# StavrosOrf/EV2Gym

Measured on AMD Instinct MI355X. Metric: env-steps/sec (envs x chargers x steps); % HBM roofline, higher is better.
Workload: dtype f64; 1 GPU; cfg2: V2GProfitPlusLoads, 50 chargers, 1 transformer, uniform[-1,1] actions; envs_per_gpu=4096, scenario_pool_per_gpu=32768, scenario_pool_order=sorted by busy window inside every window of envs_per_gpu scenarios, chargers=50, transformers=1, steps_per_episode=112, obs_dim=162, soc_log=True, launch=persistent, actor=none

## Files before the change

### ev2gym_amd/csrc/ev2g_device.h

```cpp
#pragma once
#include <hip/hip_runtime.h>
#include <stdint.h>

#define EV2G_BLOCK 256
#define EV2G_NQ 8

#include "ev2g_records.h"
typedef SessDyn PortDyn;

struct DevScn {
    int E;
    int M;
    int T, C, npc, P, R, D, ND, dt;
    int reward_kind, state_kind, flags, cost_kind;
    int n_lut;
    int G;
    int gs;
    int n_groups;
    double sixty_over_dt;
    double dt_over_60;
    const int *slot_port, *slot_cs, *slot_obs, *slot_tr;
    const int *cs_np, *cs_pbase, *slot_mask;
    const int *cs_slot0;
    int het;
// ... 853 lines not shown
    z = (z ^ (z >> 27)) * 0x94D049BB133111EBull;
    z = z ^ (z >> 31);
    return (double)(z >> 11) * (1.0 / 9007199254740992.0);
}

__global__ void ev2g_fill_uniform_kernel(double *dst, long long n, uint64_t seed, double lo, double hi) {
    for (long long i = blockIdx.x * (long long)blockDim.x + threadIdx.x; i < n; i += (long long)gridDim.x * blockDim.x)
        dst[i] = lo + (hi - lo) * ev2g_u01(seed, (uint64_t)i);
}

__device__ __forceinline__ double wave_sum(double v) {
    for (int d = 32; d > 0; d >>= 1) v += __shfl_xor(v, d, 64);
    return v;
}
__device__ __forceinline__ double wave_min(double v) {
    for (int d = 32; d > 0; d >>= 1) v = fmin(v, __shfl_xor(v, d, 64));
    return v;
}

__device__ __forceinline__ void port_sessions(const DevScn &s, const DevState &st, long long g, long long gs, int cur_step, int &first,
                                              int &last, bool &attached) {
    first = s.port_first[gs];
    last = first;
    attached = false;
    if (first < 0) return;
    const int2 w = make_int2(st.line[g].ta, st.line[g].td);
    const int cur = st.line[g].ss;
    if (cur < 0) {
        last = s.port_end[gs];
    } else {
        attached = (w.x <= cur_step);
        last = attached ? cur + 1 : cur;
    }
}

template <int EPWS> __device__ __forceinline__ double seg_sum(double v) {
    v += xor1_f64(v);
    v += xor2_f64(v);
    v += xor4_f64(v);
    v += dpp_mov_f64<0x128>(v);
    const int lo = __double2loint(v), hi = __double2hiint(v);
    const double r0 = __hiloint2double(__builtin_amdgcn_readlane(hi, 0), __builtin_amdgcn_readlane(lo, 0));
    const double r1 = __hiloint2double(__builtin_amdgcn_readlane(hi, 16), __builtin_amdgcn_readlane(lo, 16));
    const double r2 = __hiloint2double(__builtin_amdgcn_readlane(hi, 32), __builtin_amdgcn_readlane(lo, 32));
    const double r3 = __hiloint2double(__builtin_amdgcn_readlane(hi, 48), __builtin_amdgcn_readlane(lo, 48));
    if (EPWS == 1) return (r0 + r1) + (r2 + r3);
    return (threadIdx.x < 32) ? r0 + r1 : r2 + r3;
}
template <int EPWS> __device__ __forceinline__ double seg_min(double v) {
    v = fmin(v, xor1_f64(v));
    v = fmin(v, xor2_f64(v));
    v = fmin(v, xor4_f64(v));
    v = fmin(v, dpp_mov_f64<0x128>(v));
    const int lo = __double2loint(v), hi = __double2hiint(v);
    const double r0 = __hiloint2double(__builtin_amdgcn_readlane(hi, 0), __builtin_amdgcn_readlane(lo, 0));
    const double r1 = __hiloint2double(__builtin_amdgcn_readlane(hi, 16), __builtin_amdgcn_readlane(lo, 16));
    const double r2 = __hiloint2double(__builtin_amdgcn_readlane(hi, 32), __builtin_amdgcn_readlane(lo, 32));
    const double r3 = __hiloint2double(__builtin_amdgcn_readlane(hi, 48), __builtin_amdgcn_readlane(lo, 48));
    if (EPWS == 1) return fmin(fmin(r0, r1), fmin(r2, r3));
    return (threadIdx.x < 32) ? fmin(r0, r1) : fmin(r2, r3);
}
template <int EPWS> __device__ __forceinline__ bool seg_all(bool p) {
    const unsigned long long m = __ballot(p);
    if (EPWS == 1) return m == ~0ull;
    return (threadIdx.x < 32) ? ((unsigned)m == 0xffffffffu) : ((unsigned)(m >> 32) == 0xffffffffu);
}

struct StatsView {
    int T, C, R, P, dt;
    const double *setpoint;
    const int *scn_sess, *scn_sess_end, *ss_slot, *ss_tarr, *ss_tdep;
    const double *ss_B, *ss_afap;
    const int *cs_served;
    const double *cs_sat_sum, *hist, *env_acc, *sess_final_cap, *sess_abs_e, *soc_log;
    const PortLine *line;
};
__device__ __forceinline__ StatsView ev2g_stats_view(const DevScn &s, const DevState &st, const double *ss_afap) {
    return StatsView{s.T, s.C, s.R, s.P, s.dt, s.setpoint, s.scn_sess, s.scn_sess_end, s.ss_slot, s.ss_tarr, s.ss_tdep, s.ss_B, ss_afap,
                     st.cs_served, st.cs_sat_sum, st.hist, st.env_acc, st.sess_final_cap, st.sess_abs_e, st.soc_log, st.line};
}

#define EV2G_STATS_NK 40
#define EV2G_STATS_TB 8
#define EV2G_STATS_LK 16

template <int EPWS, int NK, int LK>
__device__ __forceinline__ void ev2g_env_stats(const StatsView &sv, int e, bool e_valid, int scn, int lane, int cur_step, double *__restrict__ out,
                                               double *l_keep, int lslot) {
    constexpr int W = 64 / EPWS;
    const int T = sv.T, C = sv.C, R = sv.R, P = sv.P;
    double served = 0.0, sat = 0.0, nsat = 0.0;
    for (int c = lane; c < C; c += W) {
        const int n = sv.cs_served[(long long)e * C + c];
        served += n;
        if (n > 0) { sat += sv.cs_sat_sum[(long long)e * C + c] / n; nsat += 1.0; }
    }
    served = seg_sum<EPWS>(served); sat = seg_sum<EPWS>(sat); nsat = seg_sum<EPWS>(nsat);
    double over = 0.0, te = 0.0, ete = 0.0, ptv = 0.0;
    for (int t = lane; t < T; t += W) {
        const bool past = t < cur_step;
        if (past) for (int r = 0; r < R; r++) over += sv.hist[EV2G_HIST(e, t, T, R) + 2 + r];
        const double sp = sv.setpoint[(long long)scn * T + t], u = past ? sv.hist[EV2G_HIST(e, t, T, R)] : 0.0;
        const double d = sp - u;
        te += d * d;
        ete += fabs(d);
        if (u > sp) ptv += u - sp;
    }
    over = seg_sum<EPWS>(over); te = seg_sum<EPWS>(te); ete = seg_sum<EPWS>(ete); ptv = seg_sum<EPWS>(ptv);
    ete *= (double)sv.dt / 60.0;
    if (lane == 0 && e_valid) {
        double *o = out + (long long)e * 17;
        o[0] = served;
        o[4] = (nsat > 0.0) ? sat / nsat : NAN;
        o[5] = ptv;
        o[6] = te;
        o[7] = ete;
        o[12] = over;
    }
    const double e0 = 7.543e6, e1 = 23.75e6, e2 = 6976, z0 = 7.348e-3, z1 = 3.667, z2 = 7.6e-4, z3 = 4.081e-3;
    const double b_cap_ah = 2.05, b_cap_kwh = 78, d_dist = 15000, b_age = 2 * 365, G_ = 0.186;
    const double theta = 298.15, kk = 0.8263, v_min = 3.3324;
    const double k_arrh = exp(-e2 / theta), k_age = pow(b_age, 0.25);
    const double Q_acc = 2 * (b_age * (d_dist / 365) * G_ * b_cap_ah) / b_cap_kwh, k_qacc = pow(Q_acc, 0.5);
    const bool log_soc = sv.soc_log != nullptr;
    double sum = 0.0, mn = INFINITY, cnt = 0.0, deg_cal = 0.0, deg_cyc = 0.0;
    double vkeep[2];
    int nkeep = 0;
    const int d0 = sv.scn_sess[scn], d1 = sv.scn_sess_end[scn];
    for (int k0 = d0; k0 < d1; k0 += W) {
        const int k = min(k0 + lane, d1 - 1);
        const bool has = k0 + lane < d1;
        const int q = sv.ss_slot[k], ta = sv.ss_tarr[k], td = sv.ss_tdep[k];
        const double B = sv.ss_B[k], afap = sv.ss_afap[k], fin_cap = sv.sess_final_cap[k];
        const double fin_abs = log_soc ? sv.sess_abs_e[k] : 0.0;
        const long long g = (long long)e * P + q;
        const bool spawned = has && ta <= cur_step;
        const bool live = td >= cur_step;
        const double l_cap = sv.line[g].cap, l_abs = sv.line[g].abse;
        const double capk = live ? l_cap : fin_cap;
        if (spawned) {
            const double v = capk / afap * 100.0;
            sum += v;
            mn = fmin(mn, v);
            cnt += 1.0;
            if (nkeep < 2) vkeep[nkeep] = v;
            nkeep++;
        }
        if (spawned) {
            if (log_soc) {
                const double *__restrict__ slog = sv.soc_log + (long long)e * T * P + q;
                const int tend = min(td, cur_step - 1);
                const double soc_f = capk / B;
                const double invB = 1.0 / B;
                double hs = 0.0, fs = 0.0;
                int n = 0, nf = 0;
                double xk[NK];
#pragma unroll
                for (int u = 0; u < NK; u++) xk[u] = slog[(long long)min(ta + u, tend) * P];
#pragma unroll
                for (int u = 0; u < NK; u++) {
                    if (ta + u <= tend) {
                        const double soc = fabs(xk[u]) * invB;
                        hs += soc; n++;
                        if (__double_as_longlong(xk[u]) >= 0) { fs += soc; nf++; }
                    }
                }
                for (int t = ta + NK; t <= tend; t += EV2G_STATS_TB) {
                    double x[EV2G_STATS_TB];
#pragma unroll
                    for (int u = 0; u < EV2G_STATS_TB; u++) x[u] = slog[(long long)min(t + u, tend) * P];
                    if (LK > 0 && t - ta - NK < LK) {
#pragma unroll
                        for (int u = 0; u < EV2G_STATS_TB; u++) l_keep[(t - ta - NK + u) * 64 + lslot] = x[u];
                    }
#pragma unroll
                    for (int u = 0; u < EV2G_STATS_TB; u++) {
                        if (t + u <= tend) {
                            const double soc = fabs(x[u]) * invB;
                            hs += soc; n++;
                            if (__double_as_longlong(x[u]) >= 0) { fs += soc; nf++; }
                        }
                    }
                }
                hs += soc_f; n++;
                fs += soc_f; nf++;
                const double avg_soc = hs / n, avg_f = fs / nf;
                double mad = 0.0;
#pragma unroll
                for (int u = 0; u < NK; u++)
                    if (ta + u <= tend && __double_as_longlong(xk[u]) >= 0) mad += fabs(avg_f - fabs(xk[u]) * invB);
                for (int t = ta + NK; t <= tend; t += EV2G_STATS_TB) {
                    double x[EV2G_STATS_TB];
                    if (LK > 0 && t - ta - NK < LK) {
#pragma unroll
                        for (int u = 0; u < EV2G_STATS_TB; u++) x[u] = l_keep[(t - ta - NK + u) * 64 + lslot];
                    } else {
#pragma unroll
                        for (int u = 0; u < EV2G_STATS_TB; u++) x[u] = slog[(long long)min(t + u, tend) * P];
                    }
#pragma unroll
                    for (int u = 0; u < EV2G_STATS_TB; u++)
                        if (t + u <= tend && __double_as_longlong(x[u]) >= 0) mad += fabs(avg_f - fabs(x[u]) * invB);
                }
                mad += fabs(avg_f - soc_f);
                const double delta_DoD = 2 * (mad / nf);
                const double T_sim = (td - ta + 1) * (double)sv.dt / (60 * 24);
                const double v_avg = v_min + kk * avg_soc;
                const double alpha = (e0 * v_avg - e1) * k_arrh;
                deg_cal += alpha * 0.75 * T_sim / k_age;
                const double v_half = v_min + kk * 0.5;
                const double beta = z0 * (v_half - z1) * (v_half - z1) + z2 + z3 * delta_DoD;
                const double abs_e = live ? l_abs : fin_abs;
                const double Q_sim = (abs_e / b_cap_kwh) * b_cap_ah;
                deg_cyc += beta * 0.5 * Q_sim / k_qacc;
            }
        }
    }
    sum = seg_sum<EPWS>(sum); cnt = seg_sum<EPWS>(cnt); mn = seg_min<EPWS>(mn);
    deg_cal = seg_sum<EPWS>(deg_cal); deg_cyc = seg_sum<EPWS>(deg_cyc);
    if (lane == 0 && e_valid) {
        const double *acc = sv.env_acc + (long long)e * 8;
        double *o = out + (long long)e * 17;
        o[1] = acc[1];
        o[2] = acc[2];
        o[3] = acc[3];
        o[11] = acc[4];
        o[13] = log_soc ? deg_cal + deg_cyc : NAN;
        o[14] = log_soc ? deg_cal : NAN;
        o[15] = log_soc ? deg_cyc : NAN;
        o[16] = acc[0];
    }
    double mean = NAN, sd = NAN, mnv = NAN;
    if (cnt > 0.0) {
        mean = sum / cnt;
        double var = 0.0;
        if (seg_all<EPWS>(nkeep <= 2)) {
            if (nkeep > 0) { const double v = vkeep[0] - mean; var += v * v; }
            if (nkeep > 1) { const double v = vkeep[1] - mean; var += v * v; }
        } else {
            for (int k = d0 + lane; k < d1; k += W) {
                const int ta = sv.ss_tarr[k];
                if (ta <= cur_step) {
                    const double capk = (sv.ss_tdep[k] >= cur_step) ? sv.line[(long long)e * P + sv.ss_slot[k]].cap : sv.sess_final_cap[k];
                    const double v = capk / sv.ss_afap[k] * 100.0 - mean;
                    var += v * v;
                }
            }
        }
        var = seg_sum<EPWS>(var);
        sd = sqrt(var / cnt);
        mnv = mn;
    }
    if (lane == 0 && e_valid) {
        double *o = out + (long long)e * 17;
        o[8] = mean;
        o[9] = sd;
        o[10] = mnv;
    }
}

template <int W>
__device__ __forceinline__ void ev2g_env_reset(const DevScn &s, const DevState &st, int e, int lane, int reset_off, double *__restrict__ r_obs,
                                               float *__restrict__ r_obs32) {
    const int T = s.T, C = s.C, R = s.R, P = s.P;
    const int scn_n = ev2g_scn(e, reset_off, s.M);
    const bool hfast = s.head_tab != nullptr && s.state_kind != 1 && 2 + s.head_nh <= 2 * W && (r_obs || r_obs32);
    double hrow0 = 0.0, hrow1 = 0.0;
    if (hfast) {
        const double *row = s.head_tab + (long long)scn_n * (T + 1) * s.head_nh;
        hrow0 = row[min(max(lane - 2, 0), s.head_nh - 1)];
        hrow1 = row[min(lane + W - 2, s.head_nh - 1)];
    }
    for (int q = lane; q < P; q += W) {
        const long long g = (long long)e * P + q, gs = (long long)scn_n * P + q;
        const int2 w = s.port_first_win[gs];
        st.line[g].ta = w.x; st.line[g].td = w.y; st.line[g].ss = s.port_first[gs]; st.line[g].cyc_lut = 0;
        st.line[g].cap = 0.0; st.line[g].tot = 0.0; st.line[g].prev = 0.0;
        st.port_energy[g] = 0.0; st.port_current[g] = 0.0;
        if (r_obs) { double *o = r_obs + (long long)e * s.D + s.slot_obs[q]; o[0] = 0.0; o[1] = 0.0; if (s.state_kind == 1) o[2] = 0.0; }
        if (r_obs32) { float *o = r_obs32 + (long long)e * s.D + s.slot_obs[q]; o[0] = 0.f; o[1] = 0.f; if (s.state_kind == 1) o[2] = 0.f; }
    }
    for (int c = lane; c < C; c += W) {
        const long long gc = (long long)e * C + c;
        st.cs_sat_sum[gc] = 0.0; st.cs_served[gc] = 0;
        if (st.cs_profits) { st.cs_profits[gc] = 0.0; st.cs_e_ch[gc] = 0.0; st.cs_e_dis[gc] = 0.0; st.cs_power_now[gc] = 0.0; st.cs_cur_now[gc] = 0.0; }
    }
    for (int i = lane; i < 8; i += W) st.env_acc[(long long)e * 8 + i] = 0.0;
    if (lane == 0) st.hist[EV2G_HIST(e, 0, T, R) + 1] = 0.0;
    for (int r = lane; r < R; r += W) st.tr_power_now[(long long)e * R + r] = 0.0;
    if (lane == 0) st.env_fault[e] = 0;
    if (hfast) {
        const int c0 = lane, c1 = lane + W, nc = 2 + s.head_nh;
        const double v0 = (c0 < 2) ? 0.0 : hrow0;
        if (r_obs) { double *o = r_obs + (long long)e * s.D; if (c0 < nc) o[c0] = v0; if (c1 < nc) o[c1] = hrow1; }
        if (r_obs32) { float *o = r_obs32 + (long long)e * s.D; if (c0 < nc) o[c0] = (float)v0; if (c1 < nc) o[c1] = (float)hrow1; }
    } else {
        if (r_obs) write_obs_env(s, r_obs + (long long)e * s.D, scn_n, 0, 0.0, lane, W);
        if (r_obs32) write_obs_env(s, r_obs32 + (long long)e * s.D, scn_n, 0, 0.0, lane, W);
    }
}

template <int EPWS, bool RESET = false>
__global__ void __launch_bounds__(64) ev2g_stats_kernel(DevScn s, DevState st, int scn_off,
                                                        const double *__restrict__ ss_afap, int cur_step,
                                                        double *__restrict__ out, int reset_off = 0, double *__restrict__ r_obs = nullptr,
                                                        float *__restrict__ r_obs32 = nullptr) {
    constexpr int W = 64 / EPWS;
    const int sub = threadIdx.x / W, lane = threadIdx.x - sub * W;
    const int e_raw = blockIdx.x * EPWS + sub;
    const bool e_valid = e_raw < s.E;
    const int e = e_valid ? e_raw : s.E - 1;
    const int scn = ev2g_scn(e, scn_off, s.M);
    extern __shared__ double l_keep[];
    ev2g_env_stats<EPWS, EV2G_STATS_NK, EV2G_STATS_LK>(ev2g_stats_view(s, st, ss_afap), e, e_valid, scn, lane, cur_step, out, l_keep, (int)threadIdx.x);
    if (RESET && e_valid) ev2g_env_reset<W>(s, st, e, lane, reset_off, r_obs, r_obs32);
}

template <int EPWS>
__global__ void __launch_bounds__(64) ev2g_copy_stats_reset_kernel(DevScn s, DevState st, const double *__restrict__ done_stats, double *__restrict__ out,
                                                                   int reset_off, double *__restrict__ r_obs, float *__restrict__ r_obs32) {
    constexpr int W = 64 / EPWS;
    const int sub = threadIdx.x / W, lane = threadIdx.x - sub * W;
    const int e = blockIdx.x * EPWS + sub;
    if (e >= s.E) return;
    for (int j = lane; j < 17; j += W) out[(long long)e * 17 + j] = done_stats[(long long)e * 17 + j];
    ev2g_env_reset<W>(s, st, e, lane, reset_off, r_obs, r_obs32);
}
```

### ev2gym_amd/csrc/ev2g_host.hip

```cpp
#include <hip/hip_runtime.h>

#include <algorithm>
#include <cmath>
#include <cstdio>
#include <cstring>
#include <array>
#include <map>
#include <string>
#include <utility>
#include <vector>

#include "../../include/ev2g.h"
#include "ev2g_device.h"
#include "ev2g_load_host.h"
#include "ev2g_route_host.h"
#include "ev2g_policy_host.h"
#include "ev2g_step_v2.h"
#include "ev2g_step_wave.h"
#include "ev2g_step_big.h"
#include "ev2g_mlp.h"
#include "ev2g_comm.h"
#include "ev2g_refill.h"
#include "ev2g_heuristic.h"
#include "ev2g_link.h"
// ... 78 lines not shown
    double *stat_part = nullptr, *norm_part = nullptr, *advstat = nullptr;
    PpoDev dev{};
    PpoMap map{};
    int n_blocks = 0;
    long long t = 0;
    bool have_grad = false;
};

struct ev2g_mlp;
struct ev2g_td3 : DevOwner {
    ev2g_td3_config cfg{};
    ev2g_mlp *policy = nullptr;
    Td3Plan plan;
    MlpImageMap map{};
    float lo = -1.0f;
    float *theta = nullptr, *target = nullptr, *m = nullptr, *v = nullptr, *grad = nullptr, *work = nullptr, *loss = nullptr;
    unsigned long long seed = 0, next_draw = 0;
    long long n = 0, t_critic = 0, t_actor = 0;
    int pending = 0, last_B = 0;
};
static void td3_free(ev2g_td3 *t);

struct ev2g_sac : DevOwner {
    ev2g_sac_config cfg{};
    SacPlan plan;
    SacDev dev{};
    size_t lds = 0;
    float lo = -1.0f;
    double target_entropy = 0.0;
    float *theta = nullptr, *target = nullptr, *m = nullptr, *v = nullptr, *grad = nullptr, *work = nullptr, *loss = nullptr;
    float *alpha = nullptr, *g_alpha = nullptr;
    unsigned long long seed = 0, next_draw = 0, act_seed = 0, act_n = 0;
    long long n = 0, n_target = 0, t_critic = 0, t_actor = 0;
    int pending = 0, last_B = 0, last_actor_B = 0;
};

#define EV2G_EV_RING 32
struct ev2g_handle {
    int device = 0;
    hipStream_t stream = nullptr;
    bool own_stream = false;
    ev2g_config cfg{};
    bool loaded = false;
    DevScn scn{};
    DevState st{};
    std::vector<void *> scn_allocs, st_allocs, user_allocs;
    std::vector<void *> user_host_allocs;
    void *peek_stage = nullptr; size_t peek_stage_bytes = 0;
    int E = 0, M = 0, T = 0, C = 0, npc = 0, P = 0, R = 0, D = 0;
    long long scn_off = 0;
    ev2g_step_extras extras{};
    long long S = 0;
    std::vector<int> slot_port, port_slot;
    std::vector<long long> env_sess_start;
    std::vector<int> host_to_dev;
    std::vector<int> sess_port;
    std::vector<double> sess_afap;
    long long *d_env_sess = nullptr;
    double *d_ss_afap = nullptr;
    double *d_step_tab = nullptr;
    V2P *d_v2p = nullptr;
    double *d_head_tab = nullptr; int head_nh = 0;
    double *d_lut_rowmax = nullptr;
    bool refilled = false;
    int *d_refill_overflow = nullptr;
    struct RefillCache {
        std::vector<unsigned char> key;
        std::vector<void *> allocs;
        RefillArgs args{};
    } refill_cache;
    int sess_cap = 0;
    RouteShape shape;
    StepRoute last;
    std::string big_reason;
    size_t lds_big = 0;
    BigArgs big_args{};
    std::map<ClsKey, int> cls_map;
    ClsRec *d_cls_rec = nullptr;
    std::vector<double> cs_vk_host;
    std::vector<int> cs_ph_host;
    std::vector<double> cs_imax_host;
    int load_gen = 0;
    double *d_stats_inl = nullptr;
    unsigned long long *d_ff_count = nullptr;
    int last_stats_route = -1;
    const char *stats_reason = "";
    std::string kernel_name;
    std::string fallback_reason;
    int current_step = 0;
    long long state_epoch = 0;
    size_t lds_bytes = 0;
    hipEvent_t ev0s[EV2G_EV_RING] = {}, ev1s[EV2G_EV_RING] = {};
    int ev_slot = 0;
    bool ev_valid[EV2G_EV_RING] = {};
    unsigned fused_attr_mask = 0;
    long long ev_calls = 0;
    bool timed = false;
    std::string err;
    CommState comm;
    struct RolloutGraph {
        const void *mlp; int k, t0; long long scn_off; const void *rew, *done, *mask; long long rs, ds, ms;
        ev2g_step_extras x; hipGraphExec_t exec;
    };
    std::vector<RolloutGraph> rollout_graphs;
    long long graph_launches = 0;
    int *d_port_slot = nullptr;
    double *d_heur_cs_kw = nullptr, *d_heur_cs_min_kw = nullptr;
    double heur_avg_power = 0.0, heur_min_action = 0.0;
    std::vector<ev2g_heuristic *> heuristics;
    std::vector<ev2g_link *> links;
    std::vector<ev2g_grid *> grids;
    std::vector<ev2g_wrap *> wraps;
    std::vector<ev2g_acpolicy *> acs;
    std::vector<ev2g_ppo *> ppos;
    std::vector<ev2g_td3 *> td3s;
    std::vector<ev2g_sac *> sacs;
    unsigned sac_attr_mask = 0;
    unsigned ppo_attr_mask = 0;
    unsigned ac_attr_mask = 0;
};

#define HIPCHK(h, call)                                                                              \
    do {                                                                                             \
        hipError_t e_ = (call);                                                                      \
        if (e_ != hipSuccess) {                                                                      \
            (h)->err = std::string(#call) + ": " + hipGetErrorString(e_);                            \
            return EV2G_ERR_HIP;                                                                     \
        }                                                                                            \
    } while (0)

static int fail(ev2g_handle *h, int code, const std::string &msg) {
    if (h) h->err = msg;
    else g_create_error = msg;
    return code;
}

template <typename T>
static int upload(ev2g_handle *h, std::vector<void *> &pool, const T *src, size_t n, T **dst) {
    void *p = nullptr;
    size_t bytes = std::max<size_t>(n, 1) * sizeof(T);
    HIPCHK(h, hipMalloc(&p, bytes));
    pool.push_back(p);
    if (n) HIPCHK(h, hipMemcpyAsync(p, src, n * sizeof(T), hipMemcpyHostToDevice, h->stream));
    *dst = (T *)p;
    return 0;
}
template <typename T>
static int dalloc(ev2g_handle *h, std::vector<void *> &pool, size_t n, T **dst) {
    void *p = nullptr;
    size_t bytes = std::max<size_t>(n, 1) * sizeof(T);
    HIPCHK(h, hipMalloc(&p, bytes));
    HIPCHK(h, hipMemsetAsync(p, 0, bytes, h->stream));
    pool.push_back(p);
    *dst = (T *)p;
    return 0;
}
static void state_changed(ev2g_handle *h, const char *why) {
    h->last.inl_stats = false; h->last.inl_reason = why; h->state_epoch += 1;
}

static int drain(ev2g_handle *h) {
    HIPCHK(h, hipStreamSynchronize(h->stream));
    return EV2G_OK;
}

static void free_pool(std::vector<void *> &pool) {
// ... 178 lines not shown

int ev2g_abi_version(void) { return EV2G_ABI_VERSION; }

const char *ev2g_last_error(const ev2g_handle *h) { return h ? h->err.c_str() : g_create_error.c_str(); }

int ev2g_create(const ev2g_config *cfg, ev2g_handle **out) {
    if (!cfg || !out) return fail(nullptr, EV2G_ERR_ARG, "ev2g_create: null argument");
    if (cfg->reward_kind < 0 || cfg->reward_kind >= EV2G_N_REWARDS || cfg->state_kind < 0 || cfg->state_kind > 2)
        return fail(nullptr, EV2G_ERR_ARG, "ev2g_create: unknown reward_kind/state_kind");
    if (cfg->cost_kind == EV2G_COST_TR_OVERLOAD_USRPENALTY &&
        (cfg->reward_kind == EV2G_REWARD_SQTR_TRPENALTY_USERINCENTIVES || cfg->reward_kind >= EV2G_REWARD_V2G_PROFITMAX))
        return fail(nullptr, EV2G_ERR_ARG, "ev2g_create: the fused transformer_overload_usrpenalty cost shares its per-departure staging slot with "
                                           "the user term of this reward (SqTrError_TrPenalty_UserIncentives / V2G_profitmax / *V2G_profitmaxV2): evaluate one of the two on the host");
    int n = 0;
    hipError_t e = hipGetDeviceCount(&n);
    if (e != hipSuccess || n == 0)
        return fail(nullptr, EV2G_ERR_HIP, "ev2g_create: no HIP device visible (the engine has no CPU fallback)");
    if (cfg->device < 0 || cfg->device >= n) return fail(nullptr, EV2G_ERR_ARG, "ev2g_create: device ordinal out of range");
    ev2g_handle *h = new ev2g_handle();
    h->cfg = *cfg;
    h->device = cfg->device;
    if (hipSetDevice(h->device) != hipSuccess) {
        delete h;
        return fail(nullptr, EV2G_ERR_HIP, "ev2g_create: hipSetDevice failed");
    }
    if (cfg->stream) {
        h->stream = (hipStream_t)cfg->stream;
    } else if (cfg->flags & EV2G_FLAG_NULL_STREAM) {
        h->stream = nullptr;
    } else {
        if (hipStreamCreateWithFlags(&h->stream, hipStreamNonBlocking) != hipSuccess) {
            delete h;
            return fail(nullptr, EV2G_ERR_HIP, "ev2g_create: hipStreamCreate failed");
        }
        h->own_stream = true;
    }
    for (int i = 0; i < EV2G_EV_RING; i++) { (void)hipEventCreate(&h->ev0s[i]); (void)hipEventCreate(&h->ev1s[i]); }
    *out = h;
    return EV2G_OK;
}

static void drop_rollout_graphs(ev2g_handle *h) {
    for (auto &g : h->rollout_graphs) (void)hipGraphExecDestroy(g.exec);
    h->rollout_graphs.clear();
}

void ev2g_destroy(ev2g_handle *h) {
    if (!h) return;
    (void)hipSetDevice(h->device);
    (void)hipStreamSynchronize(h->stream);
    free_pool(h->scn_allocs);
    free_pool(h->st_allocs);
    free_pool(h->user_allocs);
    for (void *p : h->user_host_allocs) (void)hipHostFree(p);
    h->user_host_allocs.clear();
    if (h->peek_stage) (void)hipHostFree(h->peek_stage);
    free_pool(h->refill_cache.allocs);
    if (h->d_refill_overflow) (void)hipFree(h->d_refill_overflow);
    release_all(h->heuristics);
    release_all(h->links);
    release_all(h->grids);
    release_all(h->wraps);
    release_all(h->ppos, ppo_free);
    release_all(h->td3s, td3_free);
    release_all(h->sacs);
    release_all(h->acs);
    ev2g_comm_destroy(h);
    drop_rollout_graphs(h);
    for (int i = 0; i < EV2G_EV_RING; i++) { if (h->ev0s[i]) (void)hipEventDestroy(h->ev0s[i]); if (h->ev1s[i]) (void)hipEventDestroy(h->ev1s[i]); }
    if (h->own_stream) (void)hipStreamDestroy(h->stream);
    delete h;
}

int ev2g_n_envs(const ev2g_handle *h) { return h ? h->E : 0; }
int ev2g_n_ports(const ev2g_handle *h) { return h ? h->P : 0; }
int ev2g_obs_dim(const ev2g_handle *h) { return h ? h->D : 0; }
int ev2g_n_steps(const ev2g_handle *h) { return h ? h->T : 0; }
int ev2g_current_step(const ev2g_handle *h) { return h ? h->current_step : 0; }
const char *ev2g_kernel_name(const ev2g_handle *h) { return (h && h->loaded) ? h->kernel_name.c_str() : ""; }
const char *ev2g_fallback_reason(const ev2g_handle *h) { return (h && h->loaded) ? h->fallback_reason.c_str() : ""; }
const char *ev2g_big_kernel_reason(const ev2g_handle *h) { return (h && h->loaded) ? h->big_reason.c_str() : ""; }
int ev2g_last_launch_specialisation(const ev2g_handle *h) { return (h && h->loaded) ? h->last.specialisation : -1; }
int ev2g_last_stats_route(const ev2g_handle *h) { return (h && h->loaded) ? h->last_stats_route : -1; }
const char *ev2g_last_stats_reason(const ev2g_handle *h) { return (h && h->loaded && h->last_stats_route == 0) ? h->stats_reason : ""; }
int ev2g_last_launch_fast_forwarded(ev2g_handle *h, int64_t *steps, int64_t *stretches) {
    if (!h || !h->loaded) return fail(h, EV2G_ERR_STATE, "ev2g_last_launch_fast_forwarded: no scenarios loaded");
    int64_t n = 0, m = 0;
    if (h->last.ff) {
        (void)hipSetDevice(h->device);
        std::vector<unsigned long long> c((size_t)h->scn.n_groups);
        HIPCHK(h, hipMemcpyAsync(c.data(), h->d_ff_count, sizeof(unsigned long long) * c.size(), hipMemcpyDeviceToHost, h->stream));
        HIPCHK(h, hipStreamSynchronize(h->stream));
        for (unsigned long long v : c) { n += (int64_t)(v & 0xffffffffull); m += (int64_t)(v >> 32); }
    }
    if (steps) *steps = n;
    if (stretches) *stretches = m;
    return EV2G_OK;
}
const char *ev2g_last_launch_general_reason(const ev2g_handle *h) { return (h && h->loaded && h->last.specialisation == 0) ? h->last.general_reason : ""; }

static const char *kStatNames[EV2G_N_STATS] = {
    "total_ev_served", "total_profits", "total_energy_charged", "total_energy_discharged",
    "average_user_satisfaction", "power_tracker_violation", "tracking_error", "energy_tracking_error",
    "energy_user_satisfaction", "std_energy_user_satisfaction", "min_energy_user_satisfaction",
    "total_steps_min_emergency_battery_capacity_violation", "total_transformer_overload",
    "battery_degradation", "battery_degradation_calendar", "battery_degradation_cycling", "total_reward"};
const char *ev2g_stat_name(int i) { return (i >= 0 && i < EV2G_N_STATS) ? kStatNames[i] : ""; }

int ev2g_reset_ex(ev2g_handle *h, double *obs, int64_t scenario_offset);

static bool stats_pair(const ev2g_handle *h) {
    const long long per_scn = h->sess_cap > 0 ? (long long)h->sess_cap : (h->S + h->M - 1) / std::max(h->M, 1);
    return (h->sess_cap > 0 ? per_scn <= 48 : h->S <= (long long)h->M * 24) && h->C <= 32;
}


static int load_route(ev2g_handle *h, const LoadPlan &p, const LoadSwitches &sw) {
    const int E = p.E, M = p.M, T = p.T, C = p.C, npc = p.npc, P = p.P, R = p.R, D = p.D, sk = h->cfg.state_kind;
    DevScn &s = h->scn;
    s = DevScn{};
    s.E = E; s.M = M; s.T = T; s.C = C; s.npc = npc; s.P = P; s.R = R; s.D = D; s.ND = std::max(p.ND, 1); s.dt = p.dt;
    s.reward_kind = h->cfg.reward_kind; s.state_kind = sk; s.flags = h->cfg.flags; s.cost_kind = h->cfg.cost_kind; s.n_lut = p.n_lut;
    s.het = p.het ? 1 : 0;
    RouteShape &rs = h->shape;
    rs = RouteShape{};
    rs.P = P; rs.T = T; rs.D = D; rs.npc = npc; rs.state_kind = sk; rs.reward_kind = h->cfg.reward_kind; rs.flags = h->cfg.flags;
    rs.block = p.het ? 0 : (P <= 256) ? 256 : (P <= 512) ? 512 : (P <= 1024) ? 1024 : 0;
    const int blk = rs.block ? rs.block : EV2G_BLOCK;
    s.G = std::max(1, blk / P);
    s.G = std::min(s.G, E);
    h->fallback_reason.clear();
    if (P < 2 || P > 64) h->fallback_reason = "ports per env outside 2..64";
    else if (R != 1) h->fallback_reason = "more than one transformer";
    else if (npc != 1) h->fallback_reason = "multi-port chargers";
    if (p.het) h->fallback_reason = "chargers with different port counts (topology file)";
    bool wave = h->fallback_reason.empty();
    rs.no_full = sw.no_full; rs.no_wide = sw.no_wide; rs.no_strided = sw.no_strided; rs.no_inl_stats = sw.no_inl_stats;
    h->last = StepRoute{}; h->last.inl_reason = "no step launch since the scenarios were loaded"; h->last_stats_route = -1;
    h->state_epoch += 1;
    if (wave) {
        const unsigned long long lim = 1ull << 32;
        const unsigned long long biggest = std::max({(unsigned long long)E * P * 8, (unsigned long long)E * D * 8,
                                                     (unsigned long long)M * (T + 1) * 60 * 8, (unsigned long long)p.SD * sizeof(SessRec),
                                                     (unsigned long long)M * T * 64, (unsigned long long)E * T * 8 * 3, (unsigned long long)M * P * 8, (unsigned long long)E * P * sizeof(PortLine),
                                                     (h->cfg.flags & EV2G_FLAG_LOG_SOC) ? (unsigned long long)E * T * P * 8 : 0ull,
                                                     (h->cfg.flags & EV2G_FLAG_LOG_CS_HISTORY) ? (unsigned long long)T * E * C * 8 : 0ull});
        if (biggest >= lim) { wave = false; h->fallback_reason = "an array of the batch reaches 4 GiB (32-bit byte offsets)"; }
    }
    if (wave && sw.kernel_v2) {
        wave = false; h->fallback_reason = "EV2G_KERNEL=v2";
    }
    rs.family = wave ? ROUTE_WAVE : rs.block ? ROUTE_V2 : ROUTE_GENERIC;
    if (wave) {
        rs.epw = 64 / P;
        s.G = (EV2G_WAVE_BLOCK / 64) * rs.epw;
        if (p.n_lut > 4094) rs.no_full = true;
    }
    {
        char nm[64];
        if (wave) std::snprintf(nm, sizeof nm, "ev2g_step_wave<%d,%d>", sk, std::min(h->cfg.reward_kind, 3));
        else if (rs.block) std::snprintf(nm, sizeof nm, "ev2g_step_v2<%d>", rs.block);
        else std::snprintf(nm, sizeof nm, "ev2g_step_kernel");
        h->kernel_name = nm;
    }
    {
        int gs = 4;
// ... 150 lines not shown
        s.win_tab = tab;
    }
    h->d_step_tab = nullptr;
    if (h->shape.wave()) {
        double *d_step_tab = nullptr;
        const size_t n = (size_t)M * T * 8;
        HIPCHK(h, hipMalloc((void **)&d_step_tab, n * sizeof(double)));
        pool.push_back(d_step_tab);
        const int nb = (int)std::min<size_t>(((size_t)M * T + 255) / 256, 4096);
        hipLaunchKernelGGL(ev2g_build_step_table_kernel, dim3(nb), dim3(256), 0, h->stream, s, d_step_tab, 0, M);
        HIPCHK(h, hipGetLastError());
        hipLaunchKernelGGL(ev2g_build_occ_mask_kernel, dim3(std::min(M, 8192)), dim3(64), 0, h->stream, s, d_step_tab, 0, M);
        HIPCHK(h, hipGetLastError());
        h->d_step_tab = d_step_tab;
    }
    h->d_head_tab = nullptr; h->head_nh = 0;
    s.head_tab = nullptr; s.head_nh = 0;
    if (h->shape.wave() && sk != EV2G_STATE_PUBLIC_PST) {
        double *d_head_tab = nullptr;
        const int NH = (sk == EV2G_STATE_V2G_PROFIT_MAX_LOADS) ? 60 : 20;
        const size_t n = (size_t)M * (T + 1) * NH;
        HIPCHK(h, hipMalloc((void **)&d_head_tab, n * sizeof(double)));
        pool.push_back(d_head_tab);
        const int nb = (int)std::min<size_t>((n + 255) / 256, 4096);
        hipLaunchKernelGGL(ev2g_build_head_table_kernel, dim3(nb), dim3(256), 0, h->stream, s.price_ch, s.win_tab, 0, M, T, NH, d_head_tab);
        HIPCHK(h, hipGetLastError());
        h->d_head_tab = d_head_tab; h->head_nh = NH;
        s.head_tab = d_head_tab; s.head_nh = NH;
    }
    return EV2G_OK;
}

static int load_alloc_state(ev2g_handle *h, long long SD) {
    const DevScn &s = h->scn;
    DevState &st = h->st;
    st = DevState{};
    auto &sp = h->st_allocs;
    const int E = s.E, T = s.T, R = s.R;
    const size_t EP = (size_t)E * s.P, EC = (size_t)E * s.C;
    int rc = 0;
#define AL(field, n) if ((rc = dalloc(h, sp, (size_t)(n), &st.field))) return rc;
    {
        AL(line, EP)
        HIPCHK(h, hipMemsetAsync(st.line, 0, EP * sizeof(PortLine), h->stream));
        if (h->shape.wave()) { AL(port_dyn, EP) }
        const size_t slice = std::max(EP, EC) * 8;
        if ((rc = dalloc(h, sp, slice * EV2G_PS_N, &st.slab_port))) return rc;
        st.slab_port_slice = slice;
#define SLICE(T, k) ((T *)(st.slab_port + slice * (size_t)(k)))
        st.port_energy = SLICE(double, EV2G_PS_PENERGY); st.port_current = SLICE(double, EV2G_PS_PCURRENT);
        st.cs_sat_sum = SLICE(double, EV2G_PS_SATSUM); st.cs_served = SLICE(int, EV2G_PS_SERVED);
#undef SLICE
    }
    if (h->cfg.flags & EV2G_FLAG_LOG_CS_HISTORY) {
        AL(cs_profits, EC) AL(cs_e_ch, EC) AL(cs_e_dis, EC) AL(cs_power_now, EC) AL(cs_cur_now, EC)
        AL(cs_power_hist, (size_t)T * EC) AL(cs_cur_hist, (size_t)T * EC)
    }
    AL(env_acc, (size_t)E * 8) AL(env_fault, E)
    AL(slab_hist, (size_t)T * E * (2 + R))
    st.hist = st.slab_hist;
    AL(slab_sess, (size_t)std::max<long long>(SD, 1) * 2)
    st.sess_final_cap = st.slab_sess;
    AL(tr_power_now, (size_t)E * R)
    if (h->cfg.flags & EV2G_FLAG_LOG_SOC) { AL(soc_log, (size_t)T * EP) st.sess_abs_e = st.slab_sess + (size_t)std::max<long long>(SD, 1); }
#ifdef EV2G_PHASE_TIMING
    AL(dbg, (size_t)s.n_groups * 18)
#endif
#undef AL
    return EV2G_OK;
}

static int load_params(ev2g_handle *h, double *d_lut_eta, V2P &v2p) {
    ev2g_v2_fill_params(v2p, h->scn, h->st);
    EV2G_SETP(v2p.lut, d_lut_eta);
    EV2G_SETP(v2p.head_tab, h->d_head_tab);
    EV2G_SETP(v2p.step_tab, h->d_step_tab);
    EV2G_SETP(v2p.ss_afap, h->d_ss_afap);
    int ex = 0;
    v2p.pow2_dt = (std::frexp(h->scn.sixty_over_dt, &ex) == 0.5 && h->scn.sixty_over_dt * h->scn.dt_over_60 == 1.0) ? 1 : 0;
    h->shape.pow2_dt = v2p.pow2_dt != 0;
    return upload(h, h->st_allocs, &v2p, 1, &h->d_v2p);
}

static int load_decide_inl_stats(ev2g_handle *h, const LoadSwitches &sw) {
    RouteShape &rs = h->shape;
    h->d_stats_inl = nullptr;
    const char *why = "";
    if (rs.no_inl_stats) why = "EV2G_NO_INLAUNCH_STATS is set";
    else if (!rs.wave() || !(h->cfg.flags & EV2G_FLAG_LOG_SOC)) why = "the step kernel is not ev2g_step_wave with the SoC log";
    else if (rs.epw != 1 || stats_pair(h)) why = "several envs per wavefront (the in-launch phase computes one env per wavefront, like the statistics kernel at this shape)";
    else if (h->lds_bytes < ev2g_inl_stats_lds_bytes()) why = "the step kernel's LDS is smaller than the phase's blocks";
    rs.inl_shape_reason = why;
    h->d_ff_count = nullptr;
    if (rs.wave() && rs.epw == 1 && !sw.no_fast_forward) {
        int rc = 0;
        if ((rc = dalloc(h, h->st_allocs, (size_t)h->scn.n_groups, &h->d_ff_count))) return rc;
        unsigned long long *p = h->d_ff_count;
        HIPCHK(h, hipMemcpy((char *)h->d_v2p + offsetof(V2P, ff_count), &p, sizeof p, hipMemcpyHostToDevice));
    }
    if (!why[0]) {
        int rc = 0;
        if ((rc = dalloc(h, h->st_allocs, (size_t)h->E * EV2G_N_STATS, &h->d_stats_inl))) return rc;
        double *p = h->d_stats_inl;
        HIPCHK(h, hipMemcpy((char *)h->d_v2p + offsetof(V2P, stats_inl), &p, sizeof p, hipMemcpyHostToDevice));
    }
    rs.ff_count = h->d_ff_count != nullptr; rs.stats_inl = h->d_stats_inl != nullptr;
    return EV2G_OK;
}

int ev2g_load_scenarios(ev2g_handle *h, const ev2g_scenario_batch *b) {
    if (!h || !b) return fail(h, EV2G_ERR_ARG, "ev2g_load_scenarios: null argument");
    (void)hipSetDevice(h->device);
    const LoadSwitches sw = load_switches_from_env();
    LoadPlan plan;
    V2P v2p;
    std::string msg;
    int rc = load_plan_check(plan, b, h->cfg, msg);
    if (rc) return fail(h, rc, msg);
    (void)hipStreamSynchronize(h->stream);
    drop_rollout_graphs(h);
    free_pool(h->scn_allocs);
    free_pool(h->st_allocs);
    h->loaded = false;
    h->cls_map.clear();

    if ((rc = load_plan_layout(plan, b, h->cfg, sw, msg))) return fail(h, rc, msg);
    h->sess_cap = (int)plan.cap;
    if ((rc = load_plan_order(plan, b, msg))) return fail(h, rc, msg);
    load_plan_constants(plan, b);
    load_plan_records(plan, b);
    if ((rc = load_route(h, plan, sw))) return rc;
    load_plan_dictionary(plan, h->shape.wave(), sw);
    if ((rc = load_route_big(h, plan, b, sw))) return rc;

    double *d_lut_eta = nullptr;
    rc = load_upload(h, plan, b, &d_lut_eta);
    if (!rc) rc = load_build_tables(h);
    if (!rc) rc = load_alloc_state(h, plan.SD);
    if (!rc) rc = load_params(h, d_lut_eta, v2p);
    if (rc) { (void)hipStreamSynchronize(h->stream); return rc; }
    HIPCHK(h, hipStreamSynchronize(h->stream));

    h->E = plan.E; h->M = plan.M; h->scn_off = 0; h->T = plan.T; h->C = plan.C; h->npc = plan.npc; h->P = plan.P; h->R = plan.R; h->D = plan.D; h->S = plan.S;
    if ((rc = load_decide_inl_stats(h, sw))) return rc;
    h->slot_port = std::move(plan.slot_port);
    h->port_slot = std::move(plan.port_slot);
    h->env_sess_start.assign(b->env_session_start, b->env_session_start + plan.M + 1);
    h->host_to_dev = std::move(plan.host_to_dev);
    h->sess_port = std::move(plan.sess_port);
    h->sess_afap = std::move(plan.sess_afap_host);
    h->cls_map = std::move(plan.cls_map);
    h->cs_vk_host = std::move(plan.cs_vk);
    h->cs_ph_host.assign(b->cs_phases, b->cs_phases + plan.C);
    h->cs_imax_host.assign(b->cs_max_charge_current, b->cs_max_charge_current + plan.C);
    h->refilled = false; h->load_gen += 1;
    h->loaded = true;
    if (h->extras.cost || h->extras.obs_f32 || h->extras.actions_f32) {
        const ev2g_step_extras keep = h->extras;
        if ((rc = ev2g_set_step_extras(h, &keep))) return rc;
    }
    return ev2g_reset_ex(h, nullptr, 0);
}

int ev2g_reset_ex(ev2g_handle *h, double *obs, int64_t scenario_offset) {
    if (!h || !h->loaded) return fail(h, EV2G_ERR_STATE, "ev2g_reset: no scenarios loaded");
    (void)hipSetDevice(h->device);
    const DevScn &s = h->scn;
    long long off = scenario_offset % (long long)s.M;
    if (off < 0) off += s.M;
    h->scn_off = off;
    if (h->st.cs_power_hist) {
        HIPCHK(h, hipMemsetAsync(h->st.cs_power_hist, 0, sizeof(double) * (size_t)s.T * s.E * s.C, h->stream));
        HIPCHK(h, hipMemsetAsync(h->st.cs_cur_hist, 0, sizeof(double) * (size_t)s.T * s.E * s.C, h->stream));
    }
    hipLaunchKernelGGL(ev2g_reset_kernel, dim3(s.n_groups), dim3(EV2G_BLOCK), 0, h->stream, s, h->st, obs, h->extras.obs_f32, (int)off);
    HIPCHK(h, hipGetLastError());
    h->current_step = 0;
    state_changed(h, "the episode was reset");
    return EV2G_OK;
}

int ev2g_reset(ev2g_handle *h, double *obs) { return ev2g_reset_ex(h, obs, h ? h->scn_off : 0); }
int ev2g_reset_f32(ev2g_handle *h, float *obs32, int64_t scenario_offset) {
    if (!h || !h->loaded) return fail(h, EV2G_ERR_STATE, "ev2g_reset: no scenarios loaded");
    const ev2g_step_extras keep = h->extras;
    if (obs32) h->extras.obs_f32 = obs32;
    const int rc = ev2g_reset_ex(h, nullptr, scenario_offset);
    h->extras = keep;
    return rc;
}
int64_t ev2g_scenario_offset(const ev2g_handle *h) { return h ? h->scn_off : 0; }
int ev2g_n_scenarios(const ev2g_handle *h) { return h ? h->M : 0; }

int ev2g_set_step_extras(ev2g_handle *h, const ev2g_step_extras *x) {
    if (!h) return EV2G_ERR_ARG;
    if (x && x->cost && h->cfg.cost_kind == EV2G_COST_NONE)
        return fail(h, EV2G_ERR_ARG, "ev2g_set_step_extras: a cost buffer needs ev2g_config.cost_kind != EV2G_COST_NONE");
    h->extras = x ? *x : ev2g_step_extras{};
    if (h->loaded && h->d_v2p) {
        (void)hipSetDevice(h->device);
        struct { void *cost; long long cs; void *o32; long long os; const void *a32; } blk{
            h->extras.cost, h->extras.cost_step_stride, h->extras.obs_f32, h->extras.obs_f32_step_stride, h->extras.actions_f32};
        static_assert(sizeof(blk) == sizeof(V2P) - offsetof(V2P, x_cost), "StepExtras block is the tail of V2P");
        HIPCHK(h, hipMemcpyAsync((char *)h->d_v2p + offsetof(V2P, x_cost), &blk, sizeof blk, hipMemcpyHostToDevice, h->stream));
        HIPCHK(h, hipStreamSynchronize(h->stream));
    }
    return EV2G_OK;
}

struct StepRows {
    Rows<const double> actions;
    Rows<double> obs, reward;
    Rows<uint8_t> done, mask;
    StepRows from(long long i) const {
        return {{actions.at(i), actions.stride}, {obs.at(i), obs.stride}, {reward.at(i), reward.stride}, {done.at(i), done.stride}, {mask.at(i), mask.stride}};
    }
};

static StepIO make_io(const ev2g_handle *h, const StepRows &r, long long step0, int auto_reset) {
    StepIO io{};
    io.actions = r.actions.p; io.a_stride = r.actions.stride;
    io.obs = r.obs.p; io.o_stride = r.obs.stride;
    io.reward = r.reward.p; io.r_stride = r.reward.stride;
    io.done = r.done.p; io.d_stride = r.done.stride;
    io.mask = r.mask.p; io.m_stride = r.mask.stride;
    io.scn_off = (int)h->scn_off;
    io.scn_stride = (auto_reset == EV2G_AUTO_RESET_NEXT) ? h->E % h->M : 0;
    io.step0 = (int)step0;
    io.log_soc = (h->cfg.flags & EV2G_FLAG_LOG_SOC) ? 1 : 0;
    io.act32 = r.actions.p ? nullptr : h->extras.actions_f32;
    io.obs32 = (h->extras.obs_f32 && h->extras.obs_f32_step_stride == 0) ? h->extras.obs_f32 : nullptr;
    return io;
}

static int launch_steps(ev2g_handle *h, const StepIO &io, int t0, int k, int auto_reset) {
    const DevScn &s = h->scn;
    const ev2g_step_extras &x = h->extras;
    h->state_epoch += 1;
    RouteCall c;
    c.actions = io.actions != nullptr; c.act32 = io.act32 != nullptr; c.obs = io.obs != nullptr; c.obs32 = io.obs32 != nullptr;
    c.reward = io.reward != nullptr; c.done = io.done != nullptr; c.mask = io.mask != nullptr;
    c.a_stride = io.a_stride; c.o_stride = io.o_stride; c.r_stride = io.r_stride; c.d_stride = io.d_stride; c.m_stride = io.m_stride;
    c.x_cost = x.cost != nullptr; c.x_obs_f32 = x.obs_f32 != nullptr; c.x_actions_f32 = x.actions_f32 != nullptr;
    c.x_cost_stride = x.cost_step_stride; c.x_obs_f32_stride = x.obs_f32_step_stride;
    c.t0 = t0; c.k = k; c.auto_reset = auto_reset;
    const StepRoute r = route_step(h->shape, c);
    if (r.refusal) {
        h->last.inl_stats = false; h->last.ff = false; h->last.inl_reason = r.inl_reason;
        return fail(h, EV2G_ERR_ARG, r.refusal);
    }
    h->last = r;
    const V2P *pp = (const V2P *)h->d_v2p;
    const LaunchDims d{dim3(s.n_groups), h->lds_bytes, h->stream};
    switch (r.family) {
    case ROUTE_WAVE: {
        const DevState &st = h->st;
        const WaveArgs wa{s.P, s.T, s.E, s.D, s.M, st.slab_port, st.slab_port_slice, st.hist,
                    st.env_acc, s.cs_pack, (char *)st.line, h->d_step_tab, (char *)st.port_dyn, s.dict, h->shape.epw, s.P};
        const WaveLaunch launch = kWaveTable[route_wave_index(r.sk, r.rk, r.io32, r.fullk)];
        if (!launch) return fail(h, EV2G_ERR_ARG, "EV2G_ONLY_00 build: only the cfg2 specialisation exists");
        launch(d, pp, io, t0, k, auto_reset, wa);
    } break;
    case ROUTE_BIG:
        hipLaunchKernelGGL(ev2g_step_big<EV2G_BIG_BLOCK>, dim3(s.E), dim3(EV2G_BIG_BLOCK), h->lds_big, h->stream, pp, io, t0, k, h->big_args);
        break;
    case ROUTE_V2:
        v2_kernel(r.block, r.spec).launch(d, pp, io, t0, k, auto_reset);
        break;
    default:
        hipLaunchKernelGGL(ev2g_step_kernel, d.grid, dim3(EV2G_BLOCK), d.lds, d.stream, s, h->st, io,
                           StepExtras{x.cost, x.cost_step_stride, x.obs_f32, x.obs_f32_step_stride, x.actions_f32}, t0, k, auto_reset);
    }
    HIPCHK(h, hipGetLastError());
    return EV2G_OK;
}

struct StepChain {
    const char *who = "";
    Rows<double> actions;
    ev2g_heuristic *agent = nullptr;
    const ev2g_mlp *actor = nullptr;
    ev2g_link *link = nullptr;
    ev2g_grid *grid = nullptr;
    double base_weight = 0.0, voltage_weight = 0.0;
    bool observed = false;
    Rows<double> vm, gobs;
    Rows<float> gobs32;
    ev2g_wrap *wrap = nullptr;
    Rows<double> wrapped;
    ev2g_acpolicy *ac = nullptr;
    bool ac_deterministic = false, ac_direct = false;
    Rows<float> ac_obs, ac_actions, ac_values, ac_log_probs;
    Rows<double> obs, reward;
    Rows<uint8_t> done, mask;
    int auto_reset = 0;
    bool a_stride_to_kernel = false;
    bool count_steps = true;
};
static int chain_steps(ev2g_handle *h, const StepChain &c, int k);
static int run_chain(ev2g_handle *h, StepChain c, int k);
static int wrap_launch(ev2g_handle *h, ev2g_wrap *w, const void *in, bool in32, double *out);
static int ac_launch(ev2g_handle *h, ev2g_acpolicy *ac, const float *x, int n_rows, bool sample, float *mean, float *actions, float *clipped,
                     float *value, float *log_prob);

int ev2g_step(ev2g_handle *h, const double *actions, double *obs, double *reward, uint8_t *done, uint8_t *action_mask) {
    if (!h || !h->loaded) return fail(h, EV2G_ERR_STATE, "ev2g_step: no scenarios loaded");
    if (!actions && !h->extras.actions_f32) return fail(h, EV2G_ERR_ARG, "ev2g_step: actions is null (and no float32 actions are set)");
    if (h->current_step >= h->T)
        return fail(h, EV2G_ERR_DONE, "ev2g_step: episode is done, reset the environment (ev2gym_env.py:343)");
    (void)hipSetDevice(h->device);
    const StepIO io = make_io(h, StepRows{{actions}, {obs}, {reward}, {done}, {action_mask}}, 0, 0);
    int rc = launch_steps(h, io, h->current_step, 1, 0);
    if (rc) return rc;
    h->current_step += 1;
    h->timed = false;
    return EV2G_OK;
}

int ev2g_step_n(ev2g_handle *h, int k_steps, int mode, const double *actions, int64_t a_stride, double *obs,
                int64_t o_stride, double *reward, int64_t r_stride, uint8_t *done, int64_t d_stride, uint8_t *mask,
                int64_t m_stride, int auto_reset) {
    if (!h || !h->loaded) return fail(h, EV2G_ERR_STATE, "ev2g_step_n: no scenarios loaded");
    if ((!actions && !h->extras.actions_f32) || k_steps < 0) return fail(h, EV2G_ERR_ARG, "ev2g_step_n: bad arguments");
    (void)hipSetDevice(h->device);
    int rc = EV2G_OK;
    const long long adv = (auto_reset == EV2G_AUTO_RESET_NEXT) ? h->E % h->M : 0;
    const StepRows rows{{actions, a_stride}, {obs, o_stride}, {reward, r_stride}, {done, d_stride}, {mask, m_stride}};
    if ((rc = timed_open(h))) return rc;
    if (mode == EV2G_STEPN_PERSISTENT) {
        int k = k_steps;
        if (!auto_reset) k = std::min(k, h->T - h->current_step);
        int resets = 0;
        { int t = h->current_step; for (int i = 0; i < k; i++) { if (t >= h->T) { t = 0; resets++; } t++; } }
        if (adv != 0 && resets > 0 && (long long)(resets + 1) * h->E > h->M) {
// ... 1998 lines not shown
    HIPCHK(h, hipStreamSynchronize(h->stream));
    return EV2G_OK;
}
int ev2g_sac_get_y(ev2g_handle *h, ev2g_sac *s, float *y, float *log_pi_next, int B) {
    if (int rc = sac_check(h, s, "ev2g_sac_get_y")) return rc;
    return sac_read_rows(h, "ev2g_sac_get_y", y, s->work + s->plan.w_y, log_pi_next, s->work + s->plan.w_lp2, B, s->last_B);
}
int ev2g_sac_get_log_pi(ev2g_handle *h, ev2g_sac *s, float *log_pi, int B) {
    if (int rc = sac_check(h, s, "ev2g_sac_get_log_pi")) return rc;
    return sac_read_rows(h, "ev2g_sac_get_log_pi", log_pi, s->work + s->plan.w_lp, nullptr, nullptr, B, s->last_actor_B);
}
int ev2g_sac_get_ent_coef(ev2g_handle *h, ev2g_sac *s, float *out3) {
    if (int rc = sac_check(h, s, "ev2g_sac_get_ent_coef")) return rc;
    if (!out3) return fail(h, EV2G_ERR_ARG, "ev2g_sac_get_ent_coef: null argument");
    HIPCHK(h, hipMemcpyAsync(out3, s->alpha, 3 * sizeof(float), hipMemcpyDeviceToHost, h->stream));
    HIPCHK(h, hipStreamSynchronize(h->stream));
    return EV2G_OK;
}
int ev2g_sac_set_rate(ev2g_handle *h, ev2g_sac *s, double lr) {
    if (int rc = sac_check(h, s, "ev2g_sac_set_rate")) return rc;
    if (int rc = fields_check(h, "ev2g_sac_set_rate", sac_rate_fields(lr))) return rc;
    s->cfg.lr = lr;
    return EV2G_OK;
}
int ev2g_sac_seed(ev2g_handle *h, ev2g_sac *s, uint64_t seed, uint64_t first_draw) {
    if (int rc = sac_check(h, s, "ev2g_sac_seed")) return rc;
    s->seed = seed; s->next_draw = first_draw;
    return EV2G_OK;
}
int ev2g_sac_act_seed(ev2g_handle *h, ev2g_sac *s, uint64_t seed, uint64_t first_launch) {
    if (int rc = sac_check(h, s, "ev2g_sac_act_seed")) return rc;
    s->act_seed = seed; s->act_n = first_launch;
    return EV2G_OK;
}
int ev2g_sac_counters(ev2g_handle *h, ev2g_sac *s, int64_t *updates, int64_t *target_updates, uint64_t *next_draw, uint64_t *act_launches) {
    if (int rc = sac_check(h, s, "ev2g_sac_counters")) return rc;
    if (updates) *updates = s->n;
    if (target_updates) *target_updates = s->n_target;
    if (next_draw) *next_draw = s->next_draw;
    if (act_launches) *act_launches = s->act_n;
    return EV2G_OK;
}

int ev2g_host_sac_head(const float *mu, const float *log_std, const float *eps, int B, int P, float lo, float *a, float *a_env, float *log_pi) {
    if (!mu || !log_std || !eps || !a || !log_pi) return fail(nullptr, EV2G_ERR_ARG, "ev2g_host_sac_head: null argument");
    if (B < 1 || P < 1) return fail(nullptr, EV2G_ERR_ARG, "ev2g_host_sac_head: B and P must be positive");
    sac_host_head(mu, log_std, eps, B, P, lo, a, a_env, log_pi);
    return EV2G_OK;
}
int ev2g_host_sac_head_back(const float *mu, const float *log_std, const float *eps, const float *g, int B, int P, float log_ent_coef, float *d_mu,
                            float *d_log_std) {
    if (!mu || !log_std || !eps || !g || !d_mu || !d_log_std) return fail(nullptr, EV2G_ERR_ARG, "ev2g_host_sac_head_back: null argument");
    if (B < 1 || P < 1) return fail(nullptr, EV2G_ERR_ARG, "ev2g_host_sac_head_back: B and P must be positive");
    sac_host_head_back(mu, log_std, eps, g, B, P, log_ent_coef, d_mu, d_log_std);
    return EV2G_OK;
}
int ev2g_host_sac_y(const float *tq, const float *log_pi_next, const float *reward, const uint8_t *done, int B, int n_critics, double gamma,
                    float log_ent_coef, float *y) {
    if (!tq || !log_pi_next || !reward || !done || !y) return fail(nullptr, EV2G_ERR_ARG, "ev2g_host_sac_y: null argument");
    if (B < 1 || n_critics < 1 || n_critics > 2) return fail(nullptr, EV2G_ERR_ARG, "ev2g_host_sac_y: B must be positive, n_critics 1 or 2");
    sac_host_y(tq, log_pi_next, reward, done, B, n_critics, gamma, log_ent_coef, y);
    return EV2G_OK;
}

int ev2g_check_faults(ev2g_handle *h, int32_t *first_bad_env) {
    if (!h || !h->loaded) return fail(h, EV2G_ERR_STATE, "ev2g_check_faults: no scenarios loaded");
    (void)hipSetDevice(h->device);
    std::vector<int> f(h->E);
    HIPCHK(h, hipMemcpyAsync(f.data(), h->st.env_fault, sizeof(int) * h->E, hipMemcpyDeviceToHost, h->stream));
    HIPCHK(h, hipStreamSynchronize(h->stream));
    for (int e = 0; e < h->E; e++)
        if (f[e]) {
            if (first_bad_env) *first_bad_env = e;
            return fail(h, EV2G_ERR_OVERCURRENT, "charger over-current: sum of amps is higher than max charge current (ev_charger.py:203-205)");
        }
    return EV2G_OK;
}

static int launch_stats(ev2g_handle *h, double *stats, bool reset, double *obs, long long off, float *obs32 = nullptr) {
    (void)hipSetDevice(h->device);
    const bool copy = h->last.inl_stats && h->current_step == h->T;
    h->last_stats_route = copy ? 1 : 0;
    h->stats_reason = copy ? "" : h->last.inl_reason;
    if (copy && !reset) {
        HIPCHK(h, hipMemcpyAsync(stats, h->d_stats_inl, sizeof(double) * (size_t)h->E * EV2G_N_STATS, hipMemcpyDeviceToDevice, h->stream));
        return EV2G_OK;
    }

    const bool pair = stats_pair(h);
    const dim3 grid(pair ? (h->E + 1) / 2 : h->E);
    if (copy) {
        hipLaunchKernelGGL((ev2g_copy_stats_reset_kernel<1>), dim3(h->E), dim3(64), 0, h->stream, h->scn, h->st, (const double *)h->d_stats_inl, stats, (int)off, obs,
                           obs32 ? obs32 : (float *)h->extras.obs_f32);
        HIPCHK(h, hipGetLastError());
        return EV2G_OK;
    }
#define EV2G_STATS_LAUNCH(EPWS, RESET)                                                                                                    \
    hipLaunchKernelGGL((ev2g_stats_kernel<EPWS, RESET>), grid, dim3(64), (size_t)EV2G_STATS_LK * 64 * sizeof(double), h->stream, h->scn, h->st, (int)h->scn_off, (const double *)h->d_ss_afap, \
                       h->current_step, stats, (int)off, obs, RESET ? (obs32 ? obs32 : (float *)h->extras.obs_f32) : (float *)nullptr)
    if (pair) { if (reset) EV2G_STATS_LAUNCH(2, true); else EV2G_STATS_LAUNCH(2, false); }
    else { if (reset) EV2G_STATS_LAUNCH(1, true); else EV2G_STATS_LAUNCH(1, false); }
#undef EV2G_STATS_LAUNCH
    HIPCHK(h, hipGetLastError());
    return EV2G_OK;
}

int ev2g_get_stats(ev2g_handle *h, double *stats) {
    if (!h || !h->loaded) return fail(h, EV2G_ERR_STATE, "ev2g_get_stats: no scenarios loaded");
    if (!stats) return fail(h, EV2G_ERR_ARG, "ev2g_get_stats: null output");
    return launch_stats(h, stats, false, nullptr, 0);
}

static int stats_reset_impl(ev2g_handle *h, double *stats, double *obs, float *obs32, int64_t scenario_offset) {
    if (!h || !h->loaded) return fail(h, EV2G_ERR_STATE, "ev2g_get_stats_reset: no scenarios loaded");
    if (!stats) return fail(h, EV2G_ERR_ARG, "ev2g_get_stats_reset: null output");
    long long off = scenario_offset % (long long)h->scn.M;
    if (off < 0) off += h->scn.M;
    const int rc = launch_stats(h, stats, true, obs, off, obs32);
    if (rc) return rc;
    if (h->st.cs_power_hist) {
        HIPCHK(h, hipMemsetAsync(h->st.cs_power_hist, 0, sizeof(double) * (size_t)h->scn.T * h->scn.E * h->scn.C, h->stream));
        HIPCHK(h, hipMemsetAsync(h->st.cs_cur_hist, 0, sizeof(double) * (size_t)h->scn.T * h->scn.E * h->scn.C, h->stream));
    }
    h->scn_off = off;
    h->current_step = 0;
    state_changed(h, "the episode was reset");
    return EV2G_OK;
}
int ev2g_get_stats_reset(ev2g_handle *h, double *stats, double *obs, int64_t scenario_offset) { return stats_reset_impl(h, stats, obs, nullptr, scenario_offset); }
int ev2g_get_stats_reset_f32(ev2g_handle *h, double *stats, float *obs32, int64_t scenario_offset) { return stats_reset_impl(h, stats, nullptr, obs32, scenario_offset); }

int ev2g_comm_get_unique_id(void *id) {
    RcclApi *api = rccl_api();
    if (!api->lib) return fail(nullptr, EV2G_ERR_STATE, "ev2g_comm_get_unique_id: " + api->err);
    if (!id) return fail(nullptr, EV2G_ERR_ARG, "ev2g_comm_get_unique_id: null output");
    static_assert(sizeof(ncclUniqueId) == EV2G_COMM_ID_BYTES, "EV2G_COMM_ID_BYTES must be sizeof(ncclUniqueId)");
    ncclUniqueId u;
    const ncclResult_t r = api->GetUniqueId(&u);
    if (r != ncclSuccess) return fail(nullptr, EV2G_ERR_HIP, std::string("ncclGetUniqueId: ") + api->GetErrorString(r));
    std::memcpy(id, &u, sizeof u);
    return EV2G_OK;
}

int ev2g_comm_init(ev2g_handle *h, const void *id, int rank, int world_size) {
    if (!h) return fail(h, EV2G_ERR_ARG, "ev2g_comm_init: null handle");
    if (!id || world_size < 1 || rank < 0 || rank >= world_size) return fail(h, EV2G_ERR_ARG, "ev2g_comm_init: bad arguments");
    RcclApi *api = rccl_api();
    if (!api->lib) return fail(h, EV2G_ERR_STATE, "ev2g_comm_init: " + api->err);
    ev2g_comm_destroy(h);
    (void)hipSetDevice(h->device);
    ncclUniqueId u;
    std::memcpy(&u, id, sizeof u);
    const ncclResult_t r = api->CommInitRank(&h->comm.comm, world_size, u, rank);
    if (r != ncclSuccess) { h->comm.comm = nullptr; return fail(h, EV2G_ERR_HIP, std::string("ncclCommInitRank: ") + api->GetErrorString(r)); }
    h->comm.rank = rank; h->comm.world = world_size;
    return EV2G_OK;
}

void ev2g_comm_destroy(ev2g_handle *h) {
    if (!h || !h->comm.comm) return;
    (void)hipSetDevice(h->device);
    (void)hipStreamSynchronize(h->stream);
    rccl_api()->CommDestroy(h->comm.comm);
    if (h->comm.d_send) (void)hipFree(h->comm.d_send);
    h->comm = CommState{};
}

int ev2g_comm_world_size(const ev2g_handle *h) { return (h && h->comm.comm) ? h->comm.world : 0; }
long long ev2g_comm_gathers(const ev2g_handle *h) { return h ? h->comm.gathers : 0; }

int ev2g_gather_stats(ev2g_handle *h, double *stats_all) {
    if (!h || !h->loaded) return fail(h, EV2G_ERR_STATE, "ev2g_gather_stats: no scenarios loaded");
    if (!h->comm.comm) return fail(h, EV2G_ERR_STATE, "ev2g_gather_stats: no communicator (call ev2g_comm_init on every rank first)");
    if (!stats_all) return fail(h, EV2G_ERR_ARG, "ev2g_gather_stats: null output");
    (void)hipSetDevice(h->device);
    if (h->comm.send_envs != h->E) {
        if (h->comm.d_send) { (void)hipStreamSynchronize(h->stream); (void)hipFree(h->comm.d_send); h->comm.d_send = nullptr; }
        HIPCHK(h, hipMalloc((void **)&h->comm.d_send, sizeof(double) * (size_t)h->E * EV2G_N_STATS));
        h->comm.send_envs = h->E;
// ... 227 lines not shown
```

### ev2gym_amd/csrc/ev2g_load_host.h

```cpp
#pragma once
#include <algorithm>
#include <array>
#include <cmath>
#include <cstdlib>
#include <cstring>
#include <map>
#include <string>
#include <utility>
#include <vector>

#include "../../include/ev2g.h"
#include "ev2g_records.h"

struct LoadSwitches {
    long long pool_session_cap = 0;
    bool no_full = false, no_wide = false, no_strided = false;
    bool no_inl_stats = false;
    bool no_fast_forward = false;
    bool kernel_v2 = false;
    bool no_dict = false;
    bool no_big = false;
};
inline LoadSwitches load_switches_from_env() {
    LoadSwitches sw;
    if (const char *e = std::getenv("EV2G_POOL_SESSION_CAP")) sw.pool_session_cap = std::atoll(e);
    sw.no_full = std::getenv("EV2G_NO_FULL") != nullptr;
    sw.no_wide = std::getenv("EV2G_NO_WIDE") != nullptr;
    sw.no_strided = std::getenv("EV2G_NO_STRIDED") != nullptr;
    sw.no_inl_stats = std::getenv("EV2G_NO_INLAUNCH_STATS") != nullptr;
    sw.no_fast_forward = std::getenv("EV2G_NO_FAST_FORWARD") != nullptr;
    const char *kn = std::getenv("EV2G_KERNEL");
    sw.kernel_v2 = kn && std::string(kn) == "v2";
    sw.no_dict = std::getenv("EV2G_NO_DICT") != nullptr;
    sw.no_big = std::getenv("EV2G_NO_BIG") != nullptr;
    return sw;
}

typedef std::array<uint64_t, 11> ClsKey;
inline int cls_find_or_add(std::map<ClsKey, int> &map, std::vector<ClsRec> &tab, const ClsRec &c) {
    ClsKey k;
    const double f[11] = {c.pacmax, c.tsm, c.gate_ch, c.B, c.rB, c.v, c.rv, c.gate_dis, c.minB, c.emerg, c.pdismax};
    std::memcpy(k.data(), f, sizeof f);
    auto it = map.find(k);
    if (it != map.end()) return it->second;
    if (map.size() >= EV2G_CLS_CAP) return -1;
    const int id = (int)map.size();
    map.emplace(k, id);
    if ((size_t)id >= tab.size()) tab.resize((size_t)id + 1);
    tab[(size_t)id] = c;
    return id;
}

inline void ev2g_sess_consts(SessRec &r, const double *vk, int cs_phases, int ev_phases, double pac_min, double pdis_min, double cs_imax) {
    const double v_gate = vk[cs_phases];
    r.gate_ch = pac_min * 1000.0 / v_gate;
    r.gate_dis = pdis_min * 1000.0 / v_gate;
    r.v = vk[std::min(cs_phases, ev_phases)];
    r.rB = 1.0 / r.B; r.rv = 1.0 / r.v;
    const double evc = r.pacmax * 1000.0 / r.v;
    r.potc = r.v * ((evc < cs_imax) ? evc : cs_imax) / 1000.0;
}

struct IntPair { int x, y; };

struct LoadPlan {
    int E = 0, M = 0, T = 0, C = 0, npc = 0, P = 0, R = 0, D = 0, ND = 0;
    int dt = 0, n_lut = 0;
    long long S = 0, SD = 0, cap = 0;
    bool het = false;
    std::vector<int> np_of, pbase;
    std::vector<int> slot_port, slot_cs, slot_tr, slot_obs, slot_mask, port_slot, cs_slot0, tr_seg, tr_obs;
    int max_seg = 1;
    std::vector<int> scn_sess, scn_sess_end;
    std::vector<int> sess_port, host_to_dev;
    std::vector<long long> dev_to_host;
    std::vector<int> ss_slot;
    std::vector<int> port_first, port_end;
    std::vector<IntPair> port_first_win;
    std::vector<int> ss_tarr, ss_tdep, ss_ntarr, ss_ntdep, ss_phases, ss_lut;
    std::vector<double> ss_cap0, ss_B, ss_des, ss_minB, ss_emerg, ss_pacmax, ss_pacmin, ss_pdismax, ss_pdismin, ss_ts, ss_tsm, ss_etach, ss_etadis;
    std::vector<double> cs_maxp, cs_minp, cs_vk, cs_dmax_abs, cs_pack;
    std::vector<double> cs_kw, cs_min_kw;
    double avg_power = 0.0, min_action = 0.0;
    std::vector<double> tr_peak, tr_base, lut_eta, rowmax;
    std::vector<double> ss_afap, sess_afap_host;
    std::vector<SessRec> recs;
    std::vector<SessTail> tails;
    std::vector<SessDyn> dyns;
    std::vector<ClsRec> cls_tab;
    std::map<ClsKey, int> cls_map;
    bool dict = false;
    std::vector<unsigned char> ccls;
    std::vector<double> ctab, ptab;
    bool many = false, even = false;
    int tmax = 0, tmin = 0;
};

inline int load_plan_check(LoadPlan &p, const ev2g_scenario_batch *b, const ev2g_config &cfg, std::string &msg) {
    const int M = b->n_envs, T = b->n_steps, C = b->n_chargers, npc = b->ports_per_charger, R = b->n_transformers;
    auto refuse = [&](const char *m) { msg = m; return EV2G_ERR_ARG; };
    p.M = M; p.T = T; p.C = C; p.npc = npc; p.R = R; p.dt = b->timescale; p.n_lut = b->n_lut;
    p.ND = std::max(b->n_dr_max, 0);
    p.E = cfg.n_active_envs > 0 ? cfg.n_active_envs : M;
    if (p.E > M) return refuse("ev2g_load_scenarios: n_active_envs exceeds the number of scenarios in the batch");
    if (M <= 0 || T <= 0 || C <= 0 || npc <= 0 || R <= 0 || b->timescale <= 0) return refuse("ev2g_load_scenarios: non-positive size");
    if (b->horizon != 20) return refuse("ev2g_load_scenarios: horizon must be 20 (state.py:119,129-132)");
    if (npc > 32) return refuse("ev2g_load_scenarios: more than 32 ports per charger unsupported");
    p.np_of.assign(C, npc); p.pbase.assign(C + 1, 0);
    p.het = false;
    if (b->cs_n_ports) {
        int mx = 0;
        for (int c = 0; c < C; c++) {
            p.np_of[c] = b->cs_n_ports[c];
            if (p.np_of[c] < 1) return refuse("ev2g_load_scenarios: cs_n_ports must be >= 1");
            mx = std::max(mx, p.np_of[c]);
            p.het = p.het || p.np_of[c] != npc;
        }
        if (mx != npc) return refuse("ev2g_load_scenarios: ports_per_charger must be the maximum of cs_n_ports");
    }
    for (int c = 0; c < C; c++) p.pbase[c + 1] = p.pbase[c] + p.np_of[c];
    const int P = p.P = p.pbase[C];
    if (p.het)
        for (int c = 0; c < C; c++)
            if (c * p.np_of[c] + p.np_of[c] > P)
                return refuse("ev2g_load_scenarios: this charger order makes the reference's action mask index "
                              "i*n_ports+j leave the mask array (ev2gym_env.py:457 raises IndexError); order the chargers by falling port count");
    const long long S = p.S = b->env_session_start[M];
    if (S != b->n_sessions || b->env_session_start[0] != 0) return refuse("ev2g_load_scenarios: env_session_start inconsistent with n_sessions");
    if (S > 0x7ffffff0LL) return refuse("ev2g_load_scenarios: too many sessions for 32-bit indices");
    {
        const long long lim = 0x7fffffffLL, Pq = P;
        const long long Dq = 3 + 3 * Pq > 22 + 40LL * R + 2 * Pq ? 3 + 3 * Pq : 22 + 40LL * R + 2 * Pq;
        const bool log_cs = (cfg.flags & EV2G_FLAG_LOG_CS_HISTORY) != 0;
        if ((long long)M * Pq > lim || (long long)M * Dq > lim || (long long)M * R * (T + 1) * 40 > lim ||
            (log_cs && (long long)T * M * std::max<long long>(C, Pq) > lim) || (long long)M * T * 8 > lim)
            return refuse("ev2g_load_scenarios: batch too large for 32-bit element offsets "
                          "(need M*P, M*D, M*R*(T+1)*40, T*M*C < 2^31): split it over more handles / GPUs");
    }
    if (T > 65535 || b->n_lut > 65534)
        return refuse("ev2g_load_scenarios: simulation_length and the number of efficiency tables must stay below 65536 (a port's state line "
                      "packs charging_cycles and the table id into 16 bits each)");
    for (int c = 0; c < C; c++) {
        if (b->cs_transformer[c] < 0 || b->cs_transformer[c] >= R) return refuse("ev2g_load_scenarios: cs_transformer out of range");
        if (b->cs_phases[c] < 1 || b->cs_phases[c] > 3) return refuse("ev2g_load_scenarios: cs_phases must be 1..3");
    }
    return EV2G_OK;
}

inline int load_plan_layout(LoadPlan &p, const ev2g_scenario_batch *b, const ev2g_config &cfg, const LoadSwitches &sw, std::string &msg) {
    const int M = p.M, C = p.C, P = p.P, R = p.R;
    for (auto *v : {&p.slot_port, &p.slot_cs, &p.slot_tr, &p.slot_obs, &p.slot_mask, &p.port_slot}) v->assign(P, 0);
    p.tr_seg.assign(R + 1, 0); p.tr_obs.assign(R, 0);
    int q = 0;
    for (int r = 0; r < R; r++) {
        p.tr_seg[r] = q;
        for (int c = 0; c < C; c++)
            if (b->cs_transformer[c] == r)
                for (int j = 0; j < p.np_of[c]; j++) {
                    p.slot_port[q] = p.pbase[c] + j;
                    p.slot_mask[q] = c * p.np_of[c] + j;
                    p.slot_cs[q] = c;
                    p.slot_tr[q] = r;
                    p.port_slot[p.pbase[c] + j] = q;
                    q++;
                }
    }
    p.tr_seg[R] = q;
    p.cs_slot0.resize(C);
    for (int c = 0; c < C; c++) p.cs_slot0[c] = p.port_slot[p.pbase[c]];
    if (cfg.state_kind == EV2G_STATE_PUBLIC_PST) {
        p.D = 3 + 3 * P;
        for (q = 0; q < P; q++) p.slot_obs[q] = 3 + 3 * q;
    } else if (cfg.state_kind == EV2G_STATE_V2G_PROFIT_MAX) {
        p.D = 22 + 2 * P;
        for (q = 0; q < P; q++) p.slot_obs[q] = 22 + 2 * q;
    } else {
        p.D = 22 + 40 * R + 2 * P;
        for (int r = 0; r < R; r++) p.tr_obs[r] = 22 + 40 * r + 2 * p.tr_seg[r];
// ... 69 lines not shown
            d++;
        }
    }
    return EV2G_OK;
}

inline double afap_energy(const ev2g_scenario_batch *b, long long s, double max_cs_power) {
    const double pac = b->ev_pac_max[s];
    const double max_power = (std::fabs(max_cs_power) > std::fabs(pac)) ? pac : max_cs_power;
    double eff;
    if (b->ev_lut[s] >= 0) {
        double m = 0;
        for (int k = 0; k < EV2G_LUT_LEN; k++) m = std::max(m, b->lut[(size_t)b->ev_lut[s] * EV2G_LUT_LEN + k]);
        eff = m / 100.0;
    } else
        eff = b->ev_eta_ch[s];
    double x = b->ev_cap0[s];
    for (int k = b->ev_t_arr[s]; k < b->ev_t_dep[s] + 1; k++) {
        x += max_power * eff * b->timescale / 60.0;
        x = std::ceil(x * 100.0) / 100.0;
        if (x > b->ev_B[s]) {
            x = b->ev_B[s];
            break;
        }
    }
    return x;
}

inline void load_plan_constants(LoadPlan &p, const ev2g_scenario_batch *b) {
    const int M = p.M, T = p.T, C = p.C, R = p.R;
    p.cs_maxp.resize(C); p.cs_minp.resize(C); p.cs_vk.resize((size_t)C * 4); p.cs_dmax_abs.resize(C);
    for (int c = 0; c < C; c++) {
        const double V = b->cs_voltage[c];
        for (int k = 0; k < 4; k++) p.cs_vk[(size_t)c * 4 + k] = V * std::sqrt((double)k);
        const double sq = std::sqrt((double)b->cs_phases[c]);
        p.cs_maxp[c] = sq * V * b->cs_max_charge_current[c] / 1000;
        p.cs_minp[c] = sq * V * b->cs_min_charge_current[c] / 1000;
        p.cs_dmax_abs[c] = std::fabs(b->cs_max_discharge_current[c]);
    }
    p.cs_kw.resize(C); p.cs_min_kw.resize(C);
    double total = 0.0;
    for (int c = 0; c < C; c++) {
        const double I = b->cs_max_charge_current[c], V = b->cs_voltage[c], sq = std::sqrt((double)b->cs_phases[c]);
        p.cs_kw[c] = I * V * sq / 1000;
        p.cs_min_kw[c] = b->cs_min_charge_current[c] * V * sq / 1000;
        total += I * V * sq / (double)p.np_of[c];
    }
    p.avg_power = total / (double)C;
    p.min_action = b->cs_min_charge_current[C - 1] / b->cs_max_charge_current[C - 1] + 1e-4;
    p.cs_pack.resize((size_t)C * 6);
    for (int c = 0; c < C; c++) {
        double *r = &p.cs_pack[(size_t)c * 6];
        r[0] = b->cs_max_charge_current[c]; r[1] = p.cs_dmax_abs[c]; r[2] = b->cs_min_charge_current[c];
        r[3] = b->cs_min_discharge_current[c]; r[4] = p.cs_maxp[c]; r[5] = p.cs_minp[c];
    }
    p.tr_peak.resize((size_t)M * R);
    for (size_t er = 0; er < (size_t)M * R; er++) {
        double m = b->tr_max_power[er * T];
        for (int t = 1; t < T; t++) m = std::max(m, b->tr_max_power[er * T + t]);
        p.tr_peak[er] = m;
    }
    p.tr_base.resize((size_t)M * R * T);
    for (size_t i = 0; i < p.tr_base.size(); i++) p.tr_base[i] = b->tr_inflexible_load[i] + b->tr_solar_power[i];
    p.lut_eta.resize((size_t)b->n_lut * EV2G_LUT_LEN);
    for (size_t i = 0; i < p.lut_eta.size(); i++) p.lut_eta[i] = b->lut[i] / 100.0;
    p.rowmax.assign((size_t)std::max(b->n_lut, 1), 0.0);
    for (int l = 0; l < b->n_lut; l++)
        for (int k = 0; k < EV2G_LUT_LEN; k++) p.rowmax[l] = std::max(p.rowmax[l], b->lut[(size_t)l * EV2G_LUT_LEN + k]);
}

inline void load_plan_records(LoadPlan &p, const ev2g_scenario_batch *b) {
    const int M = p.M;
    const long long S = p.S, SD = p.SD;
    const std::vector<long long> &dev_to_host = p.dev_to_host;
    auto gather = [&](auto &dst, const auto *src) {
        dst.assign((size_t)SD, 0);
        for (long long d = 0; d < SD; d++) if (dev_to_host[d] >= 0) dst[d] = src[dev_to_host[d]];
    };
    gather(p.ss_tarr, b->ev_t_arr); gather(p.ss_tdep, b->ev_t_dep); gather(p.ss_phases, b->ev_phases); gather(p.ss_lut, b->ev_lut);
    gather(p.ss_cap0, b->ev_cap0); gather(p.ss_B, b->ev_B); gather(p.ss_des, b->ev_desired); gather(p.ss_minB, b->ev_minB);
    gather(p.ss_emerg, b->ev_min_emerg); gather(p.ss_pacmax, b->ev_pac_max); gather(p.ss_pacmin, b->ev_pac_min);
    gather(p.ss_pdismax, b->ev_pdis_max); gather(p.ss_pdismin, b->ev_pdis_min); gather(p.ss_ts, b->ev_ts); gather(p.ss_tsm, b->ev_tsm);
    gather(p.ss_etach, b->ev_eta_ch); gather(p.ss_etadis, b->ev_eta_dis);
    p.ss_ntarr.assign((size_t)SD, EV2G_INT_MAX); p.ss_ntdep.assign((size_t)SD, EV2G_INT_MAX);
    for (long long d = 0; d + 1 < SD; d++) {
        const long long a = dev_to_host[d], c = dev_to_host[d + 1];
        if (a < 0 || c < 0) continue;
        const int64_t *st = b->env_session_start;
        const bool same_env = std::upper_bound(st, st + M + 1, (int64_t)a) == std::upper_bound(st, st + M + 1, (int64_t)c);
        if (same_env && p.sess_port[a] == p.sess_port[c]) {
            p.ss_ntarr[d] = p.ss_tarr[d + 1];
            p.ss_ntdep[d] = p.ss_tdep[d + 1];
        }
    }
    p.ss_afap.assign((size_t)SD, 0.0); p.sess_afap_host.assign((size_t)S, 0.0);
    for (long long s = 0; s < S; s++) {
        const int cs = b->ev_cs[s];
        const double mp = b->cs_max_charge_current[cs] * b->cs_voltage[cs] * std::sqrt((double)b->cs_phases[cs]) / 1000;
        p.sess_afap_host[s] = afap_energy(b, s, mp);
        p.ss_afap[p.host_to_dev[s]] = p.sess_afap_host[s];
    }
    p.recs.resize((size_t)std::max<long long>(SD, 1));
    p.tails.resize((size_t)std::max<long long>(SD, 1));
    std::memset((void *)p.recs.data(), 0, p.recs.size() * sizeof(SessRec));
    std::memset((void *)p.tails.data(), 0, p.tails.size() * sizeof(SessTail));
    for (long long d = 0; d < SD; d++) {
        const long long hs = dev_to_host[d];
        if (hs < 0) continue;
        const int cs = b->ev_cs[hs];
        SessRec &r = p.recs[d];
        r.B = p.ss_B[d]; r.cap0 = p.ss_cap0[d]; r.minB = p.ss_minB[d]; r.emerg = p.ss_emerg[d];
        r.pacmax = p.ss_pacmax[d]; r.pdismax = p.ss_pdismax[d]; r.ts = p.ss_ts[d]; r.tsm = p.ss_tsm[d];
        r.eta_ch = p.ss_etach[d]; r.eta_dis = p.ss_etadis[d];
        ev2g_sess_consts(r, &p.cs_vk[(size_t)cs * 4], b->cs_phases[cs], p.ss_phases[d], p.ss_pacmin[d], p.ss_pdismin[d], b->cs_max_charge_current[cs]);
        p.tails[d].des = p.ss_des[d]; p.tails[d].nt_arr = p.ss_ntarr[d]; p.tails[d].nt_dep = p.ss_ntdep[d];
    }
}

inline void load_plan_dictionary(LoadPlan &p, bool wave_path, const LoadSwitches &sw) {
    const long long SD = p.SD;
    p.dict = wave_path && !sw.no_dict;
    if (!wave_path) return;
    p.dyns.resize((size_t)std::max<long long>(SD, 1));
    std::memset((void *)p.dyns.data(), 0, p.dyns.size() * sizeof(SessDyn));
    for (long long d = 0; d < SD && p.dict; d++) {
        if (p.dev_to_host[d] < 0) continue;
        const int k = cls_find_or_add(p.cls_map, p.cls_tab, ev2g_cls_of(p.recs[d]));
        if (k < 0) { p.dict = false; break; }
        p.dyns[d].cls = k;
    }
    if (!p.dict) {
        p.cls_map.clear();
        p.cls_tab.assign((size_t)std::max<long long>(SD, 1), ClsRec{});
        for (long long d = 0; d < SD; d++) if (p.dev_to_host[d] >= 0) { p.cls_tab[d] = ev2g_cls_of(p.recs[d]); p.dyns[d].cls = (int)d; }
    } else
        p.cls_tab.resize(EV2G_CLS_CAP, ClsRec{});
    for (long long d = 0; d < SD; d++) {
        if (p.dev_to_host[d] < 0) continue;
        p.dyns[d].ts = p.ss_ts[d]; p.dyns[d].eta_ch = p.ss_etach[d]; p.dyns[d].eta_dis = p.ss_etadis[d]; p.dyns[d].lut = p.ss_lut[d];
    }
}

inline void load_plan_big(LoadPlan &p, const ev2g_scenario_batch *b, int ncc_max) {
    const int P = p.P;
    p.ccls.assign(P, 0); p.ctab.clear();
    p.many = false;
    for (int q = 0; q < P && !p.many; q++) {
        const int c = p.slot_cs[q];
        const double r[6] = {b->cs_max_charge_current[c], b->cs_min_charge_current[c], b->cs_min_discharge_current[c], p.cs_dmax_abs[c], p.cs_maxp[c], p.cs_minp[c]};
        int k = 0;
        const int n = (int)(p.ctab.size() / 6);
        while (k < n && std::memcmp(&p.ctab[(size_t)k * 6], r, sizeof r) != 0) k++;
        if (k == n) { if (n == ncc_max) { p.many = true; break; } p.ctab.insert(p.ctab.end(), r, r + 6); }
        p.ccls[q] = (unsigned char)k;
    }
    p.tmax = p.T; p.tmin = 0;
    for (long long d = 0; d < p.SD; d++)
        if (p.dev_to_host[d] >= 0) { p.tmax = std::max({p.tmax, p.ss_tarr[d], p.ss_tdep[d]}); p.tmin = std::min({p.tmin, p.ss_tarr[d], p.ss_tdep[d]}); }
    p.even = p.D % 2 == 0;
    for (int q = 0; q < P; q++) p.even = p.even && p.slot_obs[q] % 2 == 0;
    p.ptab.assign(15, std::nan(""));
    int npot = 0;
    for (long long d = 0; d < p.SD && npot < 15; d++) {
        if (p.dev_to_host[d] < 0) continue;
        int k = 0;
        while (k < npot && p.ptab[(size_t)k] != p.recs[d].potc) k++;
// ... 4 lines not shown
```

### ev2gym_amd/csrc/ev2g_route_host.h

```cpp
#pragma once
#include <algorithm>

#include "../../include/ev2g.h"

enum RouteFamily {
    ROUTE_GENERIC = 0,
    ROUTE_V2,
    ROUTE_BIG,
    ROUTE_WAVE
};

struct RouteShape {
    int family = ROUTE_GENERIC;
    int block = 0;
    int P = 0, T = 0, D = 0, npc = 0;
    int state_kind = 0, reward_kind = 0, flags = 0;
    bool pow2_dt = false;
    int epw = 1;
    bool no_full = false, no_wide = false, no_strided = false, no_inl_stats = false;
    bool ff_count = false;
    bool stats_inl = false;
    const char *inl_shape_reason = "";
    bool wave() const { return family == ROUTE_WAVE; }
    bool big() const { return family == ROUTE_BIG; }
};

struct RouteCall {
    bool actions = false, act32 = false, obs = false, obs32 = false, reward = false, done = false, mask = false;
    long long a_stride = 0, o_stride = 0, r_stride = 0, d_stride = 0, m_stride = 0;
    bool x_cost = false, x_obs_f32 = false, x_actions_f32 = false;
    long long x_cost_stride = 0, x_obs_f32_stride = 0;
    int t0 = 0, k = 0, auto_reset = 0;
};

struct StepRoute {
    int family = ROUTE_GENERIC;
    int sk = 0, rk = 0, fullk = 0;
    bool io32 = false;
    int block = 0;
    bool spec = false;
    int specialisation = -1;
    bool ff = false;
    bool inl_stats = false;
    const char *general_reason = "";
    const char *inl_reason = "";
    const char *refusal = nullptr;
};

inline int route_reward_slot(int reward_kind) { return std::min(reward_kind, 3); }

constexpr int ROUTE_WAVE_ENTRIES = 3 * 4 * 2 * 4;
constexpr int route_wave_index(int sk, int rk, bool io32, int fullk) { return ((sk * 4 + rk) * 2 + (io32 ? 1 : 0)) * 4 + fullk; }
constexpr bool route_wave_exists(int sk, int rk, bool io32, int fullk) {
    return sk >= 0 && sk < 3 && rk >= 0 && rk < 4 && fullk >= 0 && fullk < 4 && (fullk == 0 || (rk != 3 && (fullk != 3 || !io32)));
}

inline StepRoute route_step(const RouteShape &s, const RouteCall &c) {
    StepRoute r;
    r.inl_reason = "the step kernel is not ev2g_step_wave";
    const bool cs_hist = (s.flags & EV2G_FLAG_LOG_CS_HISTORY) != 0, log_soc = (s.flags & EV2G_FLAG_LOG_SOC) != 0;
    const bool strided = c.o_stride != 0 || c.r_stride != 0 || c.d_stride != 0 || c.m_stride != 0;
    if (s.wave()) {
        r.family = ROUTE_WAVE;
        const long long lim = 1ll << 32;
        if (c.a_stride * 8 >= lim || c.o_stride * 8 >= lim || c.r_stride * 8 >= lim || c.d_stride >= lim || c.m_stride >= lim ||
            c.x_cost_stride * 8 >= lim || c.x_obs_f32_stride * 4 >= lim || c.a_stride < 0 || c.o_stride < 0 || c.r_stride < 0 ||
            c.d_stride < 0 || c.m_stride < 0 || c.x_cost_stride < 0 || c.x_obs_f32_stride < 0) {
            r.refusal = "ev2g_step_n: a step stride is negative or reaches 4 GiB (unsupported by the fast-path kernel)";
            return r;
        }
        const int rk = route_reward_slot(s.reward_kind);
        const bool f64io = c.actions && c.obs && !c.x_obs_f32, f32io = !c.actions && c.act32 && !c.obs && c.obs32;
        const bool full0 = (f64io || f32io) && c.reward && c.done && c.mask && !c.x_cost && !cs_hist && !c.auto_reset && c.t0 + c.k <= s.T &&
                           rk != 3 && !s.no_full;
        const bool wide0 = full0 && log_soc && s.P >= 3 && !s.no_wide &&
                           s.P >= (s.state_kind == EV2G_STATE_PUBLIC_PST ? 3 : (s.state_kind == EV2G_STATE_V2G_PROFIT_MAX_LOADS ? 30 : 10));
        const bool str3 = strided && wide0 && f64io && !s.no_strided;
        const bool full = full0 && (!strided || str3), wide = wide0 && full;
        r.sk = s.state_kind; r.rk = rk;
        r.fullk = full ? (str3 ? 3 : (wide ? 2 : 1)) : 0;
        r.io32 = full ? f32io : !c.actions;
        r.specialisation = r.fullk;
        r.ff = full && !str3 && f64io && c.k > 1 && s.ff_count && s.state_kind != EV2G_STATE_PUBLIC_PST;
        if (!full) {
            if (s.no_full) r.general_reason = "EV2G_NO_FULL is set (or the batch has more than 4094 efficiency tables)";
            else if (rk == 3) r.general_reason = "the reward function is one of the eight selected at run time (only the shipped configs' three are compiled in)";
            else if (cs_hist) r.general_reason = "EV2G_FLAG_LOG_CS_HISTORY (charger histories)";
            else if (c.x_cost) r.general_reason = "a cost buffer is registered (ev2g_set_step_extras)";
            else if (c.auto_reset) r.general_reason = "auto_reset";
            else if (!(c.reward && c.done && c.mask)) r.general_reason = "a reward / done / mask output is NULL";
            else if (!(f64io || f32io)) r.general_reason = "the observation / action buffers are neither the float64 pair nor the float32 hand-over pair (e.g. obs NULL, or a float32 observation copy next to the float64 one)";
            else if (strided) r.general_reason = "an output step stride is not 0 (strided outputs keep the specialisation only with float64 observations, EV2G_FLAG_LOG_SOC and an env wide enough for the wide instantiation)";
            else r.general_reason = "the launch would run past the episode end";
        }
        if (s.no_inl_stats) r.inl_reason = "EV2G_NO_INLAUNCH_STATS is set";
        else if (c.t0 + c.k != s.T) r.inl_reason = "the last step launch did not end the episode";
        else if (c.k < 2) r.inl_reason = "the episode ended in a single-step launch (per-step launches keep the statistics kernel)";
        else if (!(wide && !str3 && f64io)) r.inl_reason = "the last step launch was not the float64 wide instantiation with step stride 0 (ev2g_last_launch_specialisation 2)";
        else if (!s.stats_inl) r.inl_reason = s.inl_shape_reason;
        else r.inl_reason = "";
        r.inl_stats = r.inl_reason[0] == 0;
        return r;
    }
    const bool v2 = s.family == ROUTE_V2 || s.family == ROUTE_BIG;
    r.spec = v2 && s.state_kind == EV2G_STATE_V2G_PROFIT_MAX_LOADS && s.reward_kind == 0 && s.npc == 1 && c.actions && c.obs && c.reward &&
             c.done && c.mask && !c.x_cost && !c.x_obs_f32 && !cs_hist && log_soc && !strided && !c.auto_reset && c.t0 + c.k <= s.T && s.pow2_dt &&
             !s.no_full;
    r.family = !v2 ? ROUTE_GENERIC : (r.spec && s.big()) ? ROUTE_BIG : ROUTE_V2;
    r.block = v2 ? s.block : 0;
    r.specialisation = v2 ? (r.spec ? (s.big() ? 5 : 1) : 0) : -1;
    return r;
}

inline bool collect_direct(const RouteShape &s, bool x_cost, bool x_obs_f32, bool x_actions_f32) {
    return s.wave() && !x_cost && !x_obs_f32 && !x_actions_f32 && !(s.flags & EV2G_FLAG_LOG_CS_HISTORY) && route_reward_slot(s.reward_kind) != 3 && !s.no_full;
}

struct FusedPacking { int ks1 = 0, nt1 = 0, nt2 = 0, nt3 = 0, nw = 0; };
struct FusedRoute {
    bool eligible = false;
    int ae = 1, nwf = 1;
    int index = -1;
};
constexpr int ROUTE_FUSED_ENTRIES = 32;
constexpr int route_fused_index(int sk, int rk, int ae, int nwf) { return nwf == 2 ? 20 + sk * 4 + rk : (ae == 2 ? 16 + rk : sk * 4 + rk); }
struct FusedKey { int sk, rk, ae, nwf; bool exists; };
constexpr FusedKey route_fused_key(int i) {
    return i < 16 ? FusedKey{i / 4, i % 4, 1, 1, i / 4 < 3 && i % 4 < 3}
         : i < 20 ? FusedKey{EV2G_STATE_PUBLIC_PST, i - 16, 2, 1, i - 16 < 3}
                  : FusedKey{(i - 20) / 4, (i - 20) % 4, 1, 2, (i - 20) / 4 < 3 && (i - 20) % 4 < 3};
}

inline FusedRoute route_fused(const RouteShape &s, bool x_cost, const FusedPacking &m, bool no_fused, bool no_fused_f32) {
    FusedRoute r;
    const bool pst = s.state_kind == EV2G_STATE_PUBLIC_PST;
    const int rk = route_reward_slot(s.reward_kind);
    r.eligible = s.wave() && s.P >= 3 && s.P <= 64 && rk != 3 && (s.flags & EV2G_FLAG_LOG_SOC) && !(s.flags & EV2G_FLAG_LOG_CS_HISTORY) && !x_cost &&
                 !s.no_full && !s.no_wide && (pst || (s.D & 1) == 0) && m.ks1 == (pst ? 2 : 6) && m.nt1 == 25 && m.nt2 == 19 && m.nt3 == (pst ? 2 : 4) &&
                 (m.nw == 1 || (m.nw == 2 && !no_fused_f32)) && !no_fused;
    r.ae = (pst && s.P <= 32 && m.nw == 1) ? 2 : 1;
    r.nwf = m.nw;
    r.index = r.eligible ? route_fused_index(s.state_kind, rk, r.ae, r.nwf) : -1;
    return r;
}
```

### ev2gym_amd/csrc/ev2g_step_v2.h

```cpp
#pragma once
#include "ev2g_device.h"

#ifdef EV2G_PHASE_TIMING
#define PT_DECL unsigned long long pt_last = __builtin_readcyclecounter(); unsigned long long pt_acc[18] = {0,0,0,0,0,0,0,0,0,0,0,0,0,0,0,0,0,0}; unsigned long long pt_cur[8] = {0,0,0,0,0,0,0,0};
#define PT_MARK(i) { unsigned long long n_ = __builtin_readcyclecounter(); pt_cur[i] += n_ - pt_last; pt_last = n_; }
#define PT_STEP_END(empty) { const int o_ = (empty) ? 8 : 0; for (int i_ = 0; i_ < 8; i_++) { pt_acc[o_ + i_] += pt_cur[i_]; pt_cur[i_] = 0; } pt_acc[16 + ((empty) ? 1 : 0)] += 1; }
#ifndef EV2G_PT_TID
#define EV2G_PT_TID 0
#endif
#define PT_FLUSH if (threadIdx.x == EV2G_PT_TID && S->dbg) { for (int i_ = 0; i_ < 8; i_++) pt_acc[i_] += pt_cur[i_]; for (int i_ = 0; i_ < 18; i_++) S->dbg[(size_t)blockIdx.x * 18 + i_] += pt_acc[i_]; }
#elif defined(EV2G_PHASE_MARKERS)
#define PT_DECL
#define PT_MARK(i) asm volatile("; PHASE_MARK " #i);
#define PT_STEP_END(empty)
#define PT_FLUSH
#else
#define PT_DECL
#define PT_MARK(i)
#define PT_STEP_END(empty)
#define PT_FLUSH
#endif

__device__ __forceinline__ void lds_barrier() { asm volatile("s_waitcnt lgkmcnt(0)\n\ts_barrier" ::: "memory"); }

// ... 29 lines not shown
        curr_soc = pilot_dsoc + soc;
        if (curr_soc > 1.0) curr_soc = 1.0;
    } else {
        const double pts = r.ts + (pilot_dsoc - max_dsoc) / max_dsoc * (r.ts - 1.0);
        const bool below = soc < pts;
        const double num = below ? r.tsm * (pilot_dsoc + soc - pts) : r.tsm * pilot_dsoc;
        const double fac = below ? (pts - 1.0) : (soc - 1.0);
        double new_soc = 1.0 + exp(num / (pts - 1.0)) * fac;
        if (below && (pilot_dsoc > 0.0 ? (pts - soc >= pilot_dsoc) : (1.0 <= (pts - soc) / pilot_dsoc))) new_soc = pilot_dsoc + soc;
        const double lim = (max_dsoc > pilot_dsoc) ? pilot_dsoc : max_dsoc;
        curr_soc = (new_soc - soc > lim) ? (lim + soc) : new_soc;
    }
    const double dsoc = curr_soc - soc;
    o.cap = curr_soc * B;
    o.energy = dsoc * B;
    o.current = ev2g_fdiv2((pow2_dt ? o.energy * sixty_over_dt : o.energy / dt_over_60) * 1000.0, v, rv);
    ev_math_finish(o, tot_e);
    return o;
}
__device__ __forceinline__ EvRes ev_math_discharge(const SessRec &r, double lutv, double amps, double cap, double prev_power, double tot_e, int cycles,
                                                   double dt, bool has_lut, double rdt, bool dt_fdiv) {
    EvRes o;
    o.cap = cap; o.prev_power = prev_power; o.tot_e = tot_e; o.energy = 0.0; o.current = 0.0; o.cycles = cycles; o.emerg = 0;
    if (amps > r.gate_dis) return o;
    if (prev_power == 0.0 || prev_power > 0.0) o.cycles = cycles + 1;
    const double v = r.v, rv = r.rv;
    double given_power = ev2g_fdiv1(amps * v, 1000.0, 1.0 / 1000.0);
    if (fabs(given_power) > fabs(r.pdismax)) given_power = r.pdismax;
    const double eta = has_lut ? lutv : r.eta_dis;
    double given_energy = ev2g_fdiv1(given_power * eta * dt, 60.0, 1.0 / 60.0);
    if (cap + given_energy < r.minB) {
        if (cap > r.minB) { o.energy = -(cap - r.minB); given_energy = o.energy; }
        else { o.energy = 0.0; given_energy = 0.0; }
        o.cap = r.minB;
    } else {
        o.energy = given_energy;
        o.cap = cap + given_energy;
    }
    if (cap > r.emerg && o.cap < r.emerg) o.emerg = 1;
    const double e60 = given_energy * 60.0;
    o.current = ev2g_fdiv2((dt_fdiv ? ev2g_fdiv1(e60, dt, rdt) : e60 / dt) * 1000.0, v, rv);
    ev_math_finish(o, tot_e);
    return o;
}

#if defined(__HIP_DEVICE_COMPILE__)
#define EV2G_GP(T) T __attribute__((address_space(1))) *
#else
#define EV2G_GP(T) T *
#endif
#define EV2G_SETP(dst, src) dst = (decltype(dst))(unsigned long long)(src)

struct V2P {
    int E, M, T, C, npc, P, R, D, G, dt, reward_kind, state_kind, cost_kind, n_lut, pow2_dt;
    int dt_fdiv;
    double sixty_over_dt, dt_over_60, rdt;
    EV2G_GP(const int) slot_cs; EV2G_GP(const int) slot_port; EV2G_GP(const int) slot_obs; EV2G_GP(const int) cs_slot0;
    EV2G_GP(const int) tr_seg; EV2G_GP(const int) tr_obs; EV2G_GP(const int) port_first;
    EV2G_GP(const int2) port_first_win;
    EV2G_GP(const double) cs_imax; EV2G_GP(const double) cs_imin; EV2G_GP(const double) cs_dmin;
    EV2G_GP(const double) cs_dmax_abs; EV2G_GP(const double) cs_maxp; EV2G_GP(const double) cs_minp;
    EV2G_GP(const double) price_ch; EV2G_GP(const double) price_dis; EV2G_GP(const double) setpoint;
    EV2G_GP(const double) tr_infl; EV2G_GP(const double) tr_solar; EV2G_GP(const double) tr_base; EV2G_GP(const double) tr_maxp;
    EV2G_GP(const double) tr_minp; EV2G_GP(const double) win_tab; EV2G_GP(const double) lut;
    EV2G_GP(const double) step_tab;
    EV2G_GP(char) slab_port; unsigned long long slab_port_slice;
    EV2G_GP(double) slab_hist; EV2G_GP(double) slab_sess; unsigned long long sess_slice;
    EV2G_GP(const double) head_tab;
    EV2G_GP(const SessRec) rec; EV2G_GP(const SessTail) tail; EV2G_GP(const int) ss_lut;
    EV2G_GP(const SessDyn) sess_dyn; EV2G_GP(const ClsRec) cls_rec;
    EV2G_GP(PortLine) line;
    EV2G_GP(double) cs_sat_sum; EV2G_GP(int) cs_served;
    EV2G_GP(double) cs_profits; EV2G_GP(double) cs_e_ch; EV2G_GP(double) cs_e_dis;
    EV2G_GP(double) cs_power_hist; EV2G_GP(double) cs_cur_hist; EV2G_GP(double) cs_power_now; EV2G_GP(double) cs_cur_now;
    EV2G_GP(double) env_acc; EV2G_GP(int) env_fault;
    EV2G_GP(double) hist; EV2G_GP(double) tr_power_now;
    EV2G_GP(double) sess_final_cap; EV2G_GP(double) port_energy; EV2G_GP(double) port_current;
    EV2G_GP(double) soc_log; EV2G_GP(double) sess_abs_e;
    EV2G_GP(unsigned long long) dbg;
    EV2G_GP(const int) scn_sess; EV2G_GP(const int) scn_sess_end; EV2G_GP(const int) ss_slot; EV2G_GP(const int) ss_tarr; EV2G_GP(const int) ss_tdep;
    EV2G_GP(const double) ss_B; EV2G_GP(const double) ss_afap;
    EV2G_GP(double) stats_inl;
    EV2G_GP(unsigned long long) ff_count;
    EV2G_GP(double) x_cost; long long x_c_stride;
    EV2G_GP(float) x_obs32; long long x_o32_stride;
    EV2G_GP(const float) x_act32;
};

inline void ev2g_v2_fill_params(V2P &p, const DevScn &s, const DevState &st) {
    p.E = s.E; p.M = s.M; p.cost_kind = s.cost_kind; p.T = s.T; p.C = s.C; p.npc = s.npc; p.P = s.P; p.R = s.R; p.D = s.D; p.G = s.G; p.dt = s.dt;
    p.reward_kind = s.reward_kind; p.state_kind = s.state_kind; p.n_lut = s.n_lut;
    p.sixty_over_dt = s.sixty_over_dt; p.dt_over_60 = s.dt_over_60;
    p.rdt = 1.0 / (double)s.dt; p.dt_fdiv = fabs(fma((double)s.dt, p.rdt, -1.0)) <= 0x1p-54 ? 1 : 0;
    EV2G_SETP(p.x_cost, (double *)nullptr); EV2G_SETP(p.x_obs32, (float *)nullptr); EV2G_SETP(p.x_act32, (const float *)nullptr);
    p.x_c_stride = 0; p.x_o32_stride = 0;
    p.pow2_dt = 0; EV2G_SETP(p.head_tab, (const double *)nullptr);
    EV2G_SETP(p.step_tab, (const double *)nullptr);
    EV2G_SETP(p.slab_port, st.slab_port); p.slab_port_slice = st.slab_port_slice;
    EV2G_SETP(p.slab_hist, st.slab_hist); EV2G_SETP(p.slab_sess, st.slab_sess);
    p.sess_slice = (unsigned long long)(st.sess_abs_e ? (st.sess_abs_e - st.slab_sess) : 0) * 8ull;
#define CPS(f) EV2G_SETP(p.f, s.f);
#define CPT(f) EV2G_SETP(p.f, st.f);
    CPS(slot_cs) CPS(slot_port) CPS(slot_obs) CPS(cs_slot0) CPS(tr_seg) CPS(tr_obs) CPS(port_first) CPS(port_first_win)
    CPS(cs_imax) CPS(cs_imin) CPS(cs_dmin) CPS(cs_dmax_abs) CPS(cs_maxp) CPS(cs_minp)
    CPS(price_ch) CPS(price_dis) CPS(setpoint) CPS(tr_infl) CPS(tr_solar) CPS(tr_base) CPS(tr_maxp) CPS(tr_minp)
    CPS(win_tab) CPS(lut) CPS(rec) CPS(tail) CPS(ss_lut) CPS(sess_dyn) CPS(cls_rec)
    CPS(scn_sess) CPS(scn_sess_end) CPS(ss_slot) CPS(ss_tarr) CPS(ss_tdep) CPS(ss_B)
    EV2G_SETP(p.ss_afap, (const double *)nullptr); EV2G_SETP(p.stats_inl, (double *)nullptr); EV2G_SETP(p.ff_count, (unsigned long long *)nullptr);
    CPT(line) CPT(cs_sat_sum) CPT(cs_served)
    CPT(cs_profits) CPT(cs_e_ch) CPT(cs_e_dis) CPT(cs_power_hist) CPT(cs_cur_hist) CPT(cs_power_now) CPT(cs_cur_now)
    CPT(env_acc) CPT(env_fault) CPT(hist) CPT(tr_power_now)
    CPT(sess_final_cap) CPT(port_energy) CPT(port_current) CPT(soc_log) CPT(sess_abs_e) CPT(dbg)
#undef CPS
#undef CPT
}

__host__ __device__ inline size_t ev2g_v2_lds_bytes(int NS, int NT, int G, int R) {
    return sizeof(double) * ((size_t)(EV2G_NQ + 7) * NS + (size_t)EV2G_NQ * NT + (size_t)EV2G_NQ * G + (size_t)NT +
                             (size_t)G * 9) +
           sizeof(int) * (6 * (size_t)NS + 2 * (size_t)R + 1 + 4);
}

#define V2C(x, c) (SPEC ? (c) : (x))
template <int BLOCK, int SPEC = 0>
__global__ void __launch_bounds__(BLOCK, 4) ev2g_step_v2(const V2P *__restrict__ params, StepIO io, int t0,
                                                         int k_steps, int auto_reset) {
    extern __shared__ double lds[];
    typedef const V2P __attribute__((address_space(4))) *ParamPtr;
    ParamPtr S = (ParamPtr)(unsigned long long)params;
    const int P = S->P, R = S->R, T = S->T, C = S->C, npc = V2C(S->npc, 1), E = S->E, D = S->D, G = S->G, M = S->M;
    int off = io.scn_off;
    int grp;
    {
        const int nb = gridDim.x, b = blockIdx.x, per = nb >> 3;
        grp = (nb & 7) == 0 ? (b & 7) * per + (b >> 3) : b;
    }
    const int e0 = grp * G;
    const int ne = min(G, E - e0);
    const int N = ne * P, NS = G * P, NT = G * R;
    double *stage = lds;
    double *s_cap = stage + (size_t)EV2G_NQ * NS;
    double *s_tot = s_cap + NS, *s_prev = s_tot + NS;
    double *s_bcap = s_prev + NS, *s_potc = s_bcap + NS;
    double *s_amps = s_potc + NS;
    double *s_abse = s_amps + NS;
    double *tsum = s_abse + NS;
    double *esum = tsum + (size_t)EV2G_NQ * NT;
    double *over_l = esum + (size_t)EV2G_NQ * G;
    double *eacc = over_l + NT;
    double *pot_prev = eacc + (size_t)G * 5;
    double *osum = pot_prev + G;
    double *pot_prev2 = osum + G;
    double *tr0max = pot_prev2 + G;
    int *s_ta = (int *)(tr0max + G);
    int *s_td = s_ta + NS, *s_ss = s_td + NS, *s_cyc = s_ss + NS;
    int *s_dirty = s_cyc + NS;
    int *items = s_dirty + NS, *seg = items + NS, *trobs = seg + R + 1, *cnt = trobs + R;
    const int tid = threadIdx.x;
    const bool log_cs = V2C(S->cs_profits != nullptr, false);
    const bool log_soc = V2C(S->soc_log != nullptr, true);
    const double dtd = (double)S->dt, sixty_over_dt = S->sixty_over_dt, dt_over_60 = S->dt_over_60;
    const bool pow2_dt = V2C(S->pow2_dt != 0, true);

    const bool valid = tid < N;
    const int el = valid ? tid / P : 0;
    const int q = valid ? tid - el * P : 0;
    const int e = e0 + el;
    const int g = e * P + q;
    const int cs = S->slot_cs[q], pref = S->slot_port[q], ocol = S->slot_obs[q];
    const double c_imax = S->cs_imax[cs], c_thr_ch = S->cs_imin[cs] - 0.01, c_dmin = S->cs_dmin[cs], c_dmaxabs = S->cs_dmax_abs[cs];
    const double c_maxp = S->cs_maxp[cs], c_minp = S->cs_minp[cs];
    int t = t0;
    if (valid) {
        const EV2G_GP(PortLine) ln = S->line + g;
        const int2 w = make_int2(ln->ta, ln->td);
        s_ta[tid] = w.x; s_td[tid] = w.y; s_ss[tid] = ln->ss; s_cyc[tid] = ev2g_line_cycles(ln->cyc_lut); s_dirty[tid] = 0;
        if (w.x <= t && t <= w.y) {
            s_cap[tid] = ln->cap; s_tot[tid] = ln->tot; s_prev[tid] = ln->prev;
            s_bcap[tid] = ln->bcap; s_potc[tid] = ln->potc;
            s_abse[tid] = log_soc ? ln->abse : 0.0;
        } else {
            s_abse[tid] = 0.0;
            s_cap[tid] = 0.0; s_tot[tid] = 0.0; s_prev[tid] = 0.0; s_bcap[tid] = 1.0; s_potc[tid] = 0.0;
        }
    }
    const int lpe = BLOCK / ne;
    const int pel = tid / lpe, pl = tid - pel * lpe;
    const bool env_lane = pel < ne;
    const int pe = e0 + (env_lane ? pel : 0);
    if (tid < 2) cnt[tid] = 0;
    for (int i = tid; i <= R; i += BLOCK) seg[i] = S->tr_seg[i];
// ... 513 lines not shown
```

### ev2gym_amd/csrc/ev2g_step_wave.h

```cpp
#pragma once
#include <type_traits>
#include "ev2g_step_v2.h"
#include "ev2g_mlp.h"

#define EV2G_WAVE_BLOCK 256
#ifndef EV2G_FF_N_MIN
#define EV2G_FF_N_MIN 1
#endif

__host__ __device__ inline size_t ev2g_wave_lds_bytes(int envs_per_group, int block = EV2G_WAVE_BLOCK) {
    const size_t NS = (size_t)block;
    return sizeof(double) * (EV2G_NQ * (NS + 8) + 7 * NS + 7 * (size_t)envs_per_group + 4 * 64) + sizeof(int) * (6 * NS + 8);
}
#define EV2G_INL_STATS_NK 12
#define EV2G_INL_STATS_LK 16
__host__ __device__ inline size_t ev2g_inl_stats_lds_bytes(int block = EV2G_WAVE_BLOCK) { return (size_t)block * EV2G_INL_STATS_LK * sizeof(double); }
#define EV2G_FUSED_BLOCK 1024
#define EV2G_FUSED_SX 200
#define EV2G_FUSED_RING 10
#define EV2G_FUSED_RING2 7

#define EV2G_FUSED_SXF 196
#define EV2G_FUSED_RINGF 4
__host__ __device__ inline size_t ev2g_fused_lds_bytes(int envs_per_wave = 1, int weight_terms = 1) {
// ... 838 lines not shown
                    stg32<double>(env_acc, a8 + 32u, n4);
                }
            }
        }
        if ((valid || hcopy) && ((F32 && out) || (!FULL && obs32))) {
            const unsigned o4 = FULL ? hb_obs_env : (unsigned)(e_l * D) * 4u;
            if (SK == 1) {
                if (q_l == 0) {
                    const float h0 = (float)((double)sstep / (double)T), h1 = (float)((sstep < T) ? pf_ob0 : 0.0), h2 = (float)usage;
                    stg32<float>(obs32, o4, h0);
                    stg32<float>(obs32, o4 + 4u, h1);
                    stg32<float>(obs32, o4 + 8u, h2);
                    if (ACT && NWF > 1) { bufXf[arow * FSXF] = h0; bufXf[arow * FSXF + 1] = h1; bufXf[arow * FSXF + 2] = h2; }
                    else
                    if (ACT) {
                        *(uint32_t *)(bufX + arow * FSX) = ev2g_pack_bf16(h0, h1);
                        bufX[arow * FSX + 2] = (uint16_t)ev2g_pack_bf16(h2, 0.f);
                    }
                }
            } else {
                if (q_l == 0) stg32<f2v>(obs32, o4, (f2v){(float)sstep, (float)usage});
                if (q_l < NPAIR) stg32<f2v>(obs32, o4 + 8u + (unsigned)q_l * 8u, (f2v){(float)pf_h0.x, (float)pf_h0.y});
                if (ACT) {
                    if (q_l == 0) xput2(0, (float)sstep, (float)usage);
                    if (q_l < NPAIR) xput2(2 + 2 * q_l, (float)pf_h0.x, (float)pf_h0.y);
                }
                if (!WIDE) {
                    if (q_l + P < NPAIR) stg32<f2v>(obs32, o4 + 8u + (unsigned)(q_l + P) * 8u, (f2v){(float)pf_h1.x, (float)pf_h1.y});
                    const unsigned h8 = (unsigned)((scn * (T + 1) + sstep) * NHEAD) * 8u;
                    for (int pi = q_l + 2 * P; pi < NPAIR; pi += P) {
                        const d2v hv = ldg32<d2v>(S->head_tab, h8 + (unsigned)pi * 16u);
                        stg32<f2v>(obs32, o4 + 8u + (unsigned)pi * 8u, (f2v){(float)hv.x, (float)hv.y});
                    }
                }
            }
        }
        if (valid && ((F64 && out) || (!FULL && obs))) {
            const unsigned o8 = FULL ? hb_obs_env : (unsigned)(e_l * D) * 8u;
            if (SK == 1) {
                if (q_l == 0) {
                    stg32<double>(obs, o8, (double)sstep / (double)T);
                    stg32<double>(obs, o8 + 8u, (sstep < T) ? pf_ob0 : 0.0);
                    stg32<double>(obs, o8 + 16u, usage);
                }
            } else {
                if (STR_NT) {
                    if (q_l == 0) stg32_nt<d2v>(obs, o8, (d2v){(double)sstep, usage});
                    if (q_l < NPAIR) stg32_nt<d2v>(obs, o8 + 16u + (unsigned)q_l * 16u, pf_h0);
                } else {
                if (q_l == 0) stg32<d2v>(obs, o8, (d2v){(double)sstep, usage});
                if (q_l < NPAIR) stg32<d2v>(obs, o8 + 16u + (unsigned)q_l * 16u, pf_h0);
                }
                if (!WIDE) {
                    if (q_l + P < NPAIR) stg32<d2v>(obs, o8 + 16u + (unsigned)(q_l + P) * 16u, pf_h1);
                    const unsigned h8 = (unsigned)((scn * (T + 1) + sstep) * NHEAD) * 8u;
                    for (int pi = q_l + 2 * P; pi < NPAIR; pi += P)
                        stg32<d2v>(obs, o8 + 16u + (unsigned)pi * 16u, ldg32<d2v>(S->head_tab, h8 + (unsigned)pi * 16u));
                }
            }
        }
        PT_MARK(5)
        PT_STEP_END(cntk[0] + cntk[1] == 0)
        t += 1;
        if (STR) { obs_run += io.o_stride; rew_run += io.r_stride; done_run += io.d_stride; mask_run += io.m_stride; }
        if (ACT) obs32_run += io.o_stride;
    }
    __syncthreads();
    if (valid) {
        const int d = s_dirty[tid];
        const unsigned g8 = (unsigned)g * 8u;
        if (d & 3) stg32<i4v>(wa.lines, l64, (i4v){FULL ? r_ta : s_ta[tid], FULL ? r_td : s_td[tid], s_ss[tid], ev2g_line_pack(s_cyc[tid], ((d >> 8) & LUTMASK) - 1)});
        if (d & 1) {
            stg32<d2v>(wa.lines, l64 + 16u, (d2v){s_cap[tid], s_tot[tid]});
            stg32<d2v>(wa.lines, l64 + 32u, (d2v){s_prev[tid], s_abse[tid]});
        }
    }
#if defined(EV2G_PHASE_TIMING) && defined(EV2G_PT_OUTER)
    asm volatile("s_waitcnt vmcnt(0)" ::: "memory");
    PT_MARK(6)
#endif
    PT_FLUSH
    double *stats_out = (INL && t == T && k_steps > 1) ? (double *)S->stats_inl : nullptr;
    if (stats_out != nullptr) {
        __syncthreads();
        const int es = e0 + wv;
        if (es < S->E) {
            const int scn_s = (int)(__builtin_amdgcn_readfirstlane(hb_step) / (64u * (unsigned)T));
            StatsView v{T, S->C, S->R, P, S->dt, (const double *)S->setpoint, (const int *)S->scn_sess, (const int *)S->scn_sess_end,
                        (const int *)S->ss_slot, (const int *)S->ss_tarr, (const int *)S->ss_tdep, (const double *)S->ss_B, (const double *)S->ss_afap,
                        (const int *)S->cs_served, (const double *)S->cs_sat_sum, (const double *)S->hist, (const double *)S->env_acc,
                        (const double *)S->sess_final_cap, (const double *)S->sess_abs_e, (const double *)S->soc_log, (const PortLine *)S->line};
            ev2g_env_stats<1, EV2G_INL_STATS_NK, EV2G_INL_STATS_LK>(v, es, true, scn_s, lane, T, stats_out,
                                                                  lds + (size_t)wv * EV2G_INL_STATS_LK * 64, lane);
        }
    }
}
```

### ev2gym_amd/engine.py

```python
from __future__ import annotations

import ctypes as C
import os
import warnings
from typing import Optional

import numpy as np

from . import _abi
from .scenario import ScenarioBatch

_LIB_PATH = os.path.join(os.path.dirname(os.path.abspath(__file__)), "libev2g_hip.so")
_lib = None


class EngineError(RuntimeError):
    def __init__(self, code, msg):
        super().__init__(f"[ev2g {code}] {msg}")
        self.code = code


def load_library(path: Optional[str] = None):
    global _lib
    if _lib is not None:
        return _lib
    path = path or os.environ.get("EV2G_LIB") or _LIB_PATH
    if os.environ.get("EV2G_NO_TORCH") != "1":
        try:
            import torch
        except ImportError:
            pass
    if not os.path.exists(path):
        raise EngineError(-2, f"{path} not found: build it with `python -m ev2gym_amd.build` "
                              "(hipcc --offload-arch=gfx950); the step engine has no CPU fallback")
    L = C.CDLL(path)
    vp, i32, i64, dbl = C.c_void_p, C.c_int32, C.c_int64, C.c_double
    protos = {
        "ev2g_abi_version": (C.c_int, []),
        "ev2g_create": (C.c_int, [C.POINTER(_abi.ConfigC), C.POINTER(vp)]),
        "ev2g_destroy": (None, [vp]),
        "ev2g_last_error": (C.c_char_p, [vp]),
        "ev2g_load_scenarios": (C.c_int, [vp, C.POINTER(_abi.ScenarioBatchC)]),
        "ev2g_n_envs": (C.c_int, [vp]), "ev2g_n_scenarios": (C.c_int, [vp]), "ev2g_n_ports": (C.c_int, [vp]), "ev2g_obs_dim": (C.c_int, [vp]),
        "ev2g_n_steps": (C.c_int, [vp]), "ev2g_current_step": (C.c_int, [vp]),
        "ev2g_reset": (C.c_int, [vp, vp]),
        "ev2g_reset_ex": (C.c_int, [vp, vp, i64]),
        "ev2g_scenario_offset": (i64, [vp]),
        "ev2g_set_step_extras": (C.c_int, [vp, C.POINTER(_abi.StepExtrasC)]),
        "ev2g_kernel_name": (C.c_char_p, [vp]),
        "ev2g_last_launch_specialisation": (C.c_int, [vp]),
        "ev2g_last_launch_general_reason": (C.c_char_p, [vp]),
        "ev2g_last_stats_route": (C.c_int, [vp]),
        "ev2g_last_stats_reason": (C.c_char_p, [vp]),
        "ev2g_last_launch_fast_forwarded": (C.c_int, [vp, C.POINTER(C.c_int64), C.POINTER(C.c_int64)]),
        "ev2g_fallback_reason": (C.c_char_p, [vp]),
        "ev2g_big_kernel_reason": (C.c_char_p, [vp]),
        "ev2g_step": (C.c_int, [vp, vp, vp, vp, vp, vp]),
        "ev2g_step_n": (C.c_int, [vp, C.c_int, C.c_int, vp, i64, vp, i64, vp, i64, vp, i64, vp, i64, C.c_int]),
        "ev2g_check_faults": (C.c_int, [vp, C.POINTER(i32)]),
        "ev2g_get_stats": (C.c_int, [vp, vp]),
        "ev2g_get_stats_reset": (C.c_int, [vp, vp, vp, C.c_int64]),
        "ev2g_get_stats_reset_f32": (C.c_int, [vp, vp, vp, C.c_int64]),
        "ev2g_reset_f32": (C.c_int, [vp, vp, C.c_int64]),
        "ev2g_collect": (C.c_int, [vp, vp, C.c_int, vp]),
        "ev2g_heuristic_create": (C.c_int, [vp, C.c_int, C.POINTER(vp)]),
        "ev2g_heuristic_destroy": (None, [vp, vp]),
        "ev2g_heuristic_actions": (C.c_int, [vp, vp, vp]),
        "ev2g_heuristic_run": (C.c_int, [vp, vp, C.c_int, vp, i64, vp, i64, vp, i64, vp, i64, vp, i64]),
        "ev2g_link_create": (C.c_int, [vp, dbl, dbl, C.c_uint64, C.c_uint64, vp, vp, C.POINTER(vp)]),
        "ev2g_link_destroy": (None, [vp, vp]),
        "ev2g_link_reset_state": (C.c_int, [vp, vp]),
        "ev2g_link_actions": (C.c_int, [vp, vp, C.c_int, vp, C.c_int, vp]),
        "ev2g_link_observe": (C.c_int, [vp, vp, C.c_int, vp, vp]),
        "ev2g_link_obs_f32": (vp, [vp, vp]),
        "ev2g_link_run": (C.c_int, [vp, vp, vp, C.c_int, vp, i64, vp, i64, vp, i64, vp, i64, vp, i64]),
        "ev2g_link_rollout": (C.c_int, [vp, vp, vp, C.c_int, vp, i64, vp, i64, vp, i64]),
        "ev2g_wrap_create": (C.c_int, [vp, C.c_int, C.POINTER(vp)]),
        "ev2g_wrap_destroy": (None, [vp, vp]),
        "ev2g_wrap_reset_state": (C.c_int, [vp, vp]),
        "ev2g_wrap_actions": (C.c_int, [vp, vp, vp, C.c_int, vp]),
        "ev2g_wrap_run": (C.c_int, [vp, vp, C.c_int, vp, i64, vp, i64, vp, i64, vp, i64, vp, i64, vp, i64]),
        "ev2g_wrap_rollout": (C.c_int, [vp, vp, vp, C.c_int, vp, i64, vp, i64, vp, i64]),
        "ev2g_grid_create": (C.c_int, [vp, C.c_int, vp, vp, dbl, dbl, C.c_int, vp, vp, C.POINTER(vp)]),
        "ev2g_grid_destroy": (None, [vp, vp]),
        "ev2g_grid_solve": (C.c_int, [vp, vp, vp, vp, C.c_int, vp, vp, vp, vp]),
        "ev2g_grid_run": (C.c_int, [vp, vp, vp, C.c_int, vp, i64, vp, i64, vp, i64, vp, i64, vp, i64, vp, i64, dbl, dbl]),
        "ev2g_grid_get_stats": (C.c_int, [vp, vp, vp, vp, vp, vp]),
        "ev2g_grid_state_attach": (C.c_int, [vp, vp, vp, C.c_int]),
        "ev2g_grid_state_dim": (C.c_int, [vp, vp]),
        "ev2g_grid_observe": (C.c_int, [vp, vp, vp, vp]),
        "ev2g_grid_run_observed": (C.c_int, [vp, vp, vp, C.c_int, vp, i64, vp, i64, vp, i64, vp, i64, vp, i64, vp, i64, dbl, dbl, vp, i64, vp, i64]),
        "ev2g_grid_rollout": (C.c_int, [vp, vp, vp, C.c_int, vp, i64, vp, i64, vp, i64, vp, i64, dbl, dbl]),
        "ev2g_ac_create": (C.c_int, [vp] + [C.c_int] * 7 + [vp] * 13 + [C.c_float, C.c_uint64, C.POINTER(vp)]),
        "ev2g_ac_destroy": (None, [vp, vp]),
        "ev2g_ac_seed": (C.c_int, [vp, vp, C.c_uint64, C.c_uint64]),
        "ev2g_ac_set_log_std": (C.c_int, [vp, vp, vp]),
        "ev2g_ac_set_weights": (C.c_int, [vp, vp] + [vp] * 12),
        "ev2g_ac_forward": (C.c_int, [vp, vp, vp, C.c_int, vp, vp]),
        "ev2g_ac_act": (C.c_int, [vp, vp, vp, C.c_int, C.c_int, vp, vp, vp, vp]),
        "ev2g_ac_collect": (C.c_int, [vp, vp, C.c_int, C.c_int, C.POINTER(_abi.OnPolicyRowsC)]),
        "ev2g_ac_host_normal": (None, [vp, i64, C.c_uint64, C.c_uint64]),
        "ev2g_gae": (C.c_int, [vp, vp, vp, vp, vp, vp, C.c_int, C.c_int, dbl, dbl, vp, vp]),
        "ev2g_host_gae": (C.c_int, [vp, vp, vp, vp, vp, C.c_int, C.c_int, dbl, dbl, vp, vp]),
        "ev2g_ppo_query": (C.c_int, [C.c_int] * 6 + [C.POINTER(_abi.PpoInfoC)]),
        "ev2g_ppo_create": (C.c_int, [vp, vp, C.POINTER(_abi.PpoConfigC), C.POINTER(vp)]),
        "ev2g_ppo_destroy": (None, [vp, vp]),
        "ev2g_ppo_set_rates": (C.c_int, [vp, vp, dbl, dbl]),
        "ev2g_ppo_grad": (C.c_int, [vp, vp] + [vp] * 6 + [C.c_int, vp]),
        "ev2g_ppo_apply": (C.c_int, [vp, vp]),
        "ev2g_ppo_minibatch": (C.c_int, [vp, vp] + [vp] * 6 + [C.c_int, vp]),
        "ev2g_ppo_get_grads": (C.c_int, [vp, vp] + [vp] * 13),
        "ev2g_ppo_sync": (C.c_int, [vp, vp]),
        "ev2g_ac_get_weights": (C.c_int, [vp, vp] + [vp] * 13),
        "ev2g_host_adam": (C.c_int, [vp, vp, vp, vp, i64, i64, dbl, dbl, dbl, dbl]),
        "ev2g_host_ppo_head": (C.c_int, [vp] * 7 + [C.c_int, C.c_int, C.POINTER(_abi.PpoConfigC), vp, vp, vp, vp]),
        "ev2g_a2c_create": (C.c_int, [vp, vp, C.POINTER(_abi.A2cConfigC), C.POINTER(vp)]),
        "ev2g_a2c_set_rate": (C.c_int, [vp, vp, dbl]),
        "ev2g_a2c_grad": (C.c_int, [vp, vp] + [vp] * 5 + [C.c_int, vp]),
        "ev2g_a2c_apply": (C.c_int, [vp, vp]),
        "ev2g_a2c_update": (C.c_int, [vp, vp] + [vp] * 5 + [C.c_int, vp]),
        "ev2g_host_rmsprop": (C.c_int, [vp, vp, vp, i64, dbl, dbl, dbl]),
        "ev2g_host_a2c_head": (C.c_int, [vp] * 6 + [C.c_int, C.c_int, C.POINTER(_abi.A2cConfigC), vp, vp, vp, vp]),
        "ev2g_td3_default_config": (C.c_int, [C.c_int, C.POINTER(_abi.Td3ConfigC)]),
        "ev2g_td3_create": (C.c_int, [vp, vp, C.POINTER(_abi.Td3ConfigC)] + [C.c_int] * 4 + [vp, vp, C.c_uint64, C.POINTER(vp)]),
        "ev2g_td3_destroy": (None, [vp, vp]),
        "ev2g_td3_update": (C.c_int, [vp, vp] + [vp] * 5 + [C.c_int, vp]),
        "ev2g_td3_critic_grad": (C.c_int, [vp, vp] + [vp] * 5 + [C.c_int, vp]),
        "ev2g_td3_actor_grad": (C.c_int, [vp, vp, vp, C.c_int, vp]),
        "ev2g_td3_apply": (C.c_int, [vp, vp]),
        "ev2g_td3_get_grads": (C.c_int, [vp, vp, vp]),
        "ev2g_td3_get_weights": (C.c_int, [vp, vp, C.c_int, vp]),
        "ev2g_td3_get_y": (C.c_int, [vp, vp, vp, C.c_int]),
        "ev2g_td3_set_rate": (C.c_int, [vp, vp, dbl]),
        "ev2g_td3_seed": (C.c_int, [vp, vp, C.c_uint64, C.c_uint64]),
        "ev2g_td3_counters": (C.c_int, [vp, vp, C.POINTER(i64), C.POINTER(i64), C.POINTER(C.c_uint64)]),
        "ev2g_replay_sample": (C.c_int, [vp, C.POINTER(_abi.ReplayRingC), C.c_int, C.c_uint64, C.c_uint64] + [vp] * 6),
        "ev2g_host_replay_indices": (C.c_int, [vp, C.c_int, C.c_int, C.c_int, C.c_int, C.c_uint64, C.c_uint64]),
        "ev2g_host_td3_target": (C.c_int, [vp] * 4 + [C.c_int] * 3 + [dbl] * 3 + [C.c_uint64, C.c_uint64, vp, vp]),
        "ev2g_host_polyak": (C.c_int, [vp, vp, i64, dbl]),
        "ev2g_sac_default_config": (C.c_int, [C.POINTER(_abi.SacConfigC)]),
        "ev2g_sac_create": (C.c_int, [vp, C.POINTER(_abi.SacConfigC)] + [C.c_int] * 4 + [C.c_float, vp, vp, C.c_uint64, C.POINTER(vp)]),
        "ev2g_sac_destroy": (None, [vp, vp]),
        "ev2g_sac_update": (C.c_int, [vp, vp] + [vp] * 5 + [C.c_int, vp]),
        "ev2g_sac_critic_grad": (C.c_int, [vp, vp] + [vp] * 5 + [C.c_int, vp]),
        "ev2g_sac_actor_grad": (C.c_int, [vp, vp, vp, C.c_int, vp]),
        "ev2g_sac_apply": (C.c_int, [vp, vp]),
        "ev2g_sac_act": (C.c_int, [vp, vp, vp, C.c_int, C.c_int, vp, vp, vp, vp]),
        "ev2g_sac_collect": (C.c_int, [vp, vp, C.c_int, C.c_int, vp]),
        "ev2g_sac_get_grads": (C.c_int, [vp, vp, vp, vp]),
        "ev2g_sac_get_weights": (C.c_int, [vp, vp, C.c_int, vp]),
        "ev2g_sac_get_y": (C.c_int, [vp, vp, vp, vp, C.c_int]),
        "ev2g_sac_get_log_pi": (C.c_int, [vp, vp, vp, C.c_int]),
        "ev2g_sac_get_ent_coef": (C.c_int, [vp, vp, vp]),
        "ev2g_sac_set_rate": (C.c_int, [vp, vp, dbl]),
        "ev2g_sac_seed": (C.c_int, [vp, vp, C.c_uint64, C.c_uint64]),
        "ev2g_sac_act_seed": (C.c_int, [vp, vp, C.c_uint64, C.c_uint64]),
        "ev2g_sac_counters": (C.c_int, [vp, vp, C.POINTER(i64), C.POINTER(i64), C.POINTER(C.c_uint64), C.POINTER(C.c_uint64)]),
        "ev2g_host_sac_head": (C.c_int, [vp, vp, vp, C.c_int, C.c_int, C.c_float, vp, vp, vp]),
        "ev2g_host_sac_head_back": (C.c_int, [vp, vp, vp, vp, C.c_int, C.c_int, C.c_float, vp, vp]),
        "ev2g_host_sac_y": (C.c_int, [vp, vp, vp, vp, C.c_int, C.c_int, dbl, C.c_float, vp]),
        "ev2g_stat_name": (C.c_char_p, [C.c_int]),
        "ev2g_peek": (C.c_int, [vp, C.c_int, C.POINTER(_abi.EnvViewC)]),
        "ev2g_malloc": (vp, [vp, C.c_size_t]),
        "ev2g_free": (None, [vp, vp]),
        "ev2g_memcpy_h2d": (C.c_int, [vp, vp, vp, C.c_size_t]),
        "ev2g_memcpy_d2h": (C.c_int, [vp, vp, vp, C.c_size_t]),
        "ev2g_host_malloc": (vp, [vp, C.c_size_t]),
        "ev2g_host_free": (None, [vp, vp]),
        "ev2g_synchronize": (C.c_int, [vp]),
        "ev2g_fill_uniform": (C.c_int, [vp, vp, i64, C.c_uint64, dbl, dbl]),
        "ev2g_host_uniform": (None, [vp, i64, C.c_uint64, dbl, dbl]),
        "ev2g_last_step_n_kernel_ms": (dbl, [vp]),
        "ev2g_mlp_create": (C.c_int, [vp, C.c_int, C.c_int, C.c_int, C.c_int, vp, vp, vp, vp, vp, vp, C.c_float, C.POINTER(vp)]),
        "ev2g_mlp_create_ex": (C.c_int, [vp, C.c_int, C.c_int, C.c_int, C.c_int, vp, vp, vp, vp, vp, vp, C.c_float, C.c_int, C.POINTER(vp)]),
        "ev2g_mlp_destroy": (None, [vp, vp]),
        "ev2g_mlp_forward": (C.c_int, [vp, vp, vp, vp, C.c_int]),
        "ev2g_mlp_kernel_name": (C.c_char_p, [vp]),
        "ev2g_rollout": (C.c_int, [vp, vp, C.c_int, vp, i64, vp, i64, vp, i64, C.c_int]),
        "ev2g_rollout_graph_launches": (C.c_longlong, [vp]),
        "ev2g_comm_get_unique_id": (C.c_int, [vp]),
        "ev2g_comm_init": (C.c_int, [vp, vp, C.c_int, C.c_int]),
        "ev2g_comm_destroy": (None, [vp]),
        "ev2g_step_n_kernel_ms_back": (dbl, [vp, C.c_int]),
        "ev2g_comm_world_size": (C.c_int, [vp]),
        "ev2g_comm_gathers": (C.c_longlong, [vp]),
        "ev2g_gather_stats": (C.c_int, [vp, vp]),
        "ev2g_pool_refill": (C.c_int, [vp, C.POINTER(_abi.GenConfigC), C.c_uint64, i64, i32, i32]),
        "ev2g_pool_refill_overflows": (C.c_longlong, [vp]),
        "ev2g_pool_session_capacity": (C.c_int, [vp]),
        "ev2g_gen_default_config": (C.c_int, [C.c_int, C.POINTER(_abi.GenConfigC)]),
        "ev2g_generate": (C.c_int, [C.POINTER(_abi.GenConfigC), i32, C.c_uint64, i32, C.POINTER(vp)]),
        "ev2g_gen_batch": (C.POINTER(_abi.ScenarioBatchC), [vp]),
        "ev2g_gen_free": (None, [vp]),
        "ev2g_gen_table": (C.c_int, [C.c_int, C.c_int, C.POINTER(C.c_double), C.c_int]),
    }
    for name, (res, args) in protos.items():
        fn = getattr(L, name)
        fn.restype = res
        fn.argtypes = args
    if L.ev2g_abi_version() != _abi.ABI_VERSION:
        raise EngineError(-1, "libev2g_hip.so ABI version mismatch")
    _lib = L
    return L


EXPORTED_SYMBOLS = [
    "ev2g_abi_version", "ev2g_create", "ev2g_destroy", "ev2g_last_error", "ev2g_load_scenarios", "ev2g_n_envs",
    "ev2g_n_scenarios", "ev2g_n_ports", "ev2g_obs_dim", "ev2g_n_steps", "ev2g_current_step", "ev2g_reset", "ev2g_reset_ex",
    "ev2g_scenario_offset", "ev2g_set_step_extras", "ev2g_kernel_name", "ev2g_last_launch_specialisation", "ev2g_last_launch_general_reason", "ev2g_last_stats_route", "ev2g_last_stats_reason", "ev2g_last_launch_fast_forwarded", "ev2g_fallback_reason", "ev2g_big_kernel_reason", "ev2g_step", "ev2g_step_n",
    "ev2g_check_faults", "ev2g_get_stats", "ev2g_get_stats_reset", "ev2g_get_stats_reset_f32", "ev2g_reset_f32", "ev2g_collect", "ev2g_stat_name", "ev2g_peek", "ev2g_malloc", "ev2g_free",
    "ev2g_memcpy_h2d", "ev2g_memcpy_d2h", "ev2g_host_malloc", "ev2g_host_free", "ev2g_synchronize", "ev2g_fill_uniform", "ev2g_host_uniform",
    "ev2g_last_step_n_kernel_ms", "ev2g_step_n_kernel_ms_back", "ev2g_mlp_create", "ev2g_mlp_create_ex", "ev2g_mlp_destroy", "ev2g_mlp_forward", "ev2g_mlp_kernel_name", "ev2g_rollout",
    "ev2g_rollout_graph_launches", "ev2g_comm_get_unique_id", "ev2g_comm_init", "ev2g_comm_destroy", "ev2g_comm_world_size", "ev2g_comm_gathers", "ev2g_gather_stats",
    "ev2g_pool_refill", "ev2g_pool_refill_overflows", "ev2g_pool_session_capacity", "ev2g_gen_default_config", "ev2g_generate", "ev2g_gen_batch", "ev2g_gen_free", "ev2g_gen_table",
    "ev2g_heuristic_create", "ev2g_heuristic_destroy", "ev2g_heuristic_actions", "ev2g_heuristic_run",
    "ev2g_link_create", "ev2g_link_destroy", "ev2g_link_reset_state", "ev2g_link_actions", "ev2g_link_observe", "ev2g_link_obs_f32",
    "ev2g_link_run", "ev2g_link_rollout",
    "ev2g_grid_create", "ev2g_grid_destroy", "ev2g_grid_solve", "ev2g_grid_run",
    "ev2g_grid_state_attach", "ev2g_grid_state_dim", "ev2g_grid_observe", "ev2g_grid_run_observed", "ev2g_grid_rollout", "ev2g_grid_get_stats",
    "ev2g_wrap_create", "ev2g_wrap_destroy", "ev2g_wrap_reset_state", "ev2g_wrap_actions", "ev2g_wrap_run", "ev2g_wrap_rollout",
    "ev2g_ac_create", "ev2g_ac_destroy", "ev2g_ac_seed", "ev2g_ac_set_log_std", "ev2g_ac_set_weights", "ev2g_ac_forward", "ev2g_ac_act",
    "ev2g_ac_collect", "ev2g_ac_host_normal", "ev2g_gae", "ev2g_host_gae",
    "ev2g_ppo_query", "ev2g_ppo_create", "ev2g_ppo_destroy", "ev2g_ppo_set_rates", "ev2g_ppo_grad", "ev2g_ppo_apply", "ev2g_ppo_minibatch",
    "ev2g_ppo_get_grads", "ev2g_ppo_sync", "ev2g_ac_get_weights", "ev2g_host_adam", "ev2g_host_ppo_head",
    "ev2g_a2c_create", "ev2g_a2c_set_rate", "ev2g_a2c_grad", "ev2g_a2c_apply", "ev2g_a2c_update", "ev2g_host_rmsprop", "ev2g_host_a2c_head",
    "ev2g_td3_default_config", "ev2g_td3_create", "ev2g_td3_destroy", "ev2g_td3_update", "ev2g_td3_critic_grad", "ev2g_td3_actor_grad", "ev2g_td3_apply",
    "ev2g_td3_get_grads", "ev2g_td3_get_weights", "ev2g_td3_get_y", "ev2g_td3_set_rate", "ev2g_td3_seed", "ev2g_td3_counters", "ev2g_replay_sample",
    "ev2g_host_replay_indices", "ev2g_host_td3_target", "ev2g_host_polyak",
    "ev2g_sac_default_config", "ev2g_sac_create", "ev2g_sac_destroy", "ev2g_sac_update", "ev2g_sac_critic_grad", "ev2g_sac_actor_grad", "ev2g_sac_apply",
    "ev2g_sac_act", "ev2g_sac_collect", "ev2g_sac_get_grads", "ev2g_sac_get_weights", "ev2g_sac_get_y", "ev2g_sac_get_log_pi", "ev2g_sac_get_ent_coef",
    "ev2g_sac_set_rate", "ev2g_sac_seed", "ev2g_sac_act_seed", "ev2g_sac_counters", "ev2g_host_sac_head", "ev2g_host_sac_head_back", "ev2g_host_sac_y"]


def _ptr(x):
    if x is None:
        return None
    if isinstance(x, DeviceBuffer):
        return x.ptr
    if hasattr(x, "data_ptr"):
        return int(x.data_ptr())
    return int(x)


class DeviceBuffer:

    def __init__(self, engine: "Engine", shape, dtype):
        self.engine = engine
        self.shape = tuple(int(s) for s in np.atleast_1d(shape))
        self.dtype = np.dtype(dtype)
        self.nbytes = int(np.prod(self.shape)) * self.dtype.itemsize
        self.ptr = engine._lib.ev2g_malloc(engine._h, self.nbytes)
        if not self.ptr:
            raise EngineError(-2, engine.last_error())

    def upload(self, arr):
        arr = np.ascontiguousarray(arr, self.dtype)
        assert arr.nbytes == self.nbytes, (arr.shape, self.shape)
        self.engine._check(self.engine._lib.ev2g_memcpy_h2d(self.engine._h, self.ptr, arr.ctypes.data, self.nbytes))
        return self

    def to_host(self, out=None):
        if out is None:
            out = np.empty(self.shape, self.dtype)
        else:
            assert out.dtype == self.dtype and out.nbytes == self.nbytes and out.flags.c_contiguous
        self.engine._check(self.engine._lib.ev2g_memcpy_d2h(self.engine._h, out.ctypes.data, self.ptr, self.nbytes))
        return out

    def at(self, index_elems: int):
        return self.ptr + int(index_elems) * self.dtype.itemsize

    def free(self):
        if self.ptr and self.engine._h:
            self.engine._lib.ev2g_free(self.engine._h, self.ptr)
        self.ptr = None


class Engine:

    def __init__(self, batch: ScenarioBatch, reward_kind: int, state_kind: int, device: int = 0, flags: int = 0,
                 stream: Optional[int] = None, cost_kind: int = 0, n_active_envs: int = 0):
        self._lib = load_library()
        self._h = None
        self._spec_checks_left = 4
        cfg = _abi.ConfigC(int(device), int(reward_kind), int(state_kind), int(flags), stream, int(cost_kind), int(n_active_envs))
        h = C.c_void_p()
        rc = self._lib.ev2g_create(C.byref(cfg), C.byref(h))
        if rc != 0:
            raise EngineError(rc, (self._lib.ev2g_last_error(None) or b"").decode())
        self._h = h
        self.reward_kind, self.state_kind, self.flags, self.device = reward_kind, state_kind, flags, device
        self.load(batch)

    def load(self, batch: ScenarioBatch):
        cb = batch.to_c()
        self._check(self._lib.ev2g_load_scenarios(self._h, C.byref(cb)))
        self.batch = batch
        self.E = self._lib.ev2g_n_envs(self._h)
        self.M = self._lib.ev2g_n_scenarios(self._h)
        self.P = self._lib.ev2g_n_ports(self._h)
        self.D = self._lib.ev2g_obs_dim(self._h)
        self.T = self._lib.ev2g_n_steps(self._h)
        self.C, self.R = batch.n_chargers, batch.n_transformers
        why = self.fallback_reason
        if why and self.P <= 64:
            import warnings
            warnings.warn(f"ev2gym_amd: step kernel {self.kernel_name} selected instead of the fast path ({why})", stacklevel=2)

    @property
    def kernel_name(self) -> str:
        return (self._lib.ev2g_kernel_name(self._h) or b"").decode()

    @property
    def last_launch_specialisation(self) -> int:
        return int(self._lib.ev2g_last_launch_specialisation(self._h))

    @property
    def last_stats_route(self) -> int:
        return int(self._lib.ev2g_last_stats_route(self._h))

    @property
    def last_stats_reason(self) -> str:
        return (self._lib.ev2g_last_stats_reason(self._h) or b"").decode()

    @property
    def last_launch_fast_forwarded(self):
        n, m = C.c_int64(0), C.c_int64(0)
        self._check(self._lib.ev2g_last_launch_fast_forwarded(self._h, C.byref(n), C.byref(m)))
        return int(n.value), int(m.value)

    @property
    def fallback_reason(self) -> str:
        return (self._lib.ev2g_fallback_reason(self._h) or b"").decode()

    @property
    def big_kernel_reason(self) -> str:
        return (self._lib.ev2g_big_kernel_reason(self._h) or b"").decode()

    @property
    def scenario_offset(self) -> int:
        return int(self._lib.ev2g_scenario_offset(self._h))

    def set_extras(self, cost=None, cost_stride=0, obs_f32=None, obs_f32_stride=0, actions_f32=None):
        self._extras_keep = (cost, obs_f32, actions_f32)
        x = _abi.StepExtrasC(_ptr(cost), int(cost_stride), _ptr(obs_f32), int(obs_f32_stride), _ptr(actions_f32))
        self._check(self._lib.ev2g_set_step_extras(self._h, C.byref(x)))

    def last_error(self) -> str:
        return (self._lib.ev2g_last_error(self._h) or b"").decode()

    def _check(self, rc):
        if rc != 0:
            raise EngineError(rc, self.last_error())

    def empty(self, shape, dtype=np.float64) -> DeviceBuffer:
        return DeviceBuffer(self, shape, dtype)

    def pinned(self, shape, dtype=np.float64) -> np.ndarray:
        dt = np.dtype(dtype)
        n = int(np.prod(shape)) * dt.itemsize
        p = self._lib.ev2g_host_malloc(self._h, max(n, 1))
        if not p:
            raise EngineError("ev2g_host_malloc failed")
        buf = (C.c_char * max(n, 1)).from_address(p)
        return np.frombuffer(buf, dtype=dt, count=int(np.prod(shape))).reshape(shape)

    def memcpy_d2h(self, host_array: np.ndarray, dev_ptr, nbytes: int):
        assert host_array.flags.c_contiguous and host_array.nbytes >= nbytes
        self._check(self._lib.ev2g_memcpy_d2h(self._h, host_array.ctypes.data, _ptr(dev_ptr), int(nbytes)))

    def synchronize(self):
        self._check(self._lib.ev2g_synchronize(self._h))

    @property
    def current_step(self) -> int:
        return self._lib.ev2g_current_step(self._h)

    def reset(self, obs=None, offset: Optional[int] = None):
        if offset is None:
            self._check(self._lib.ev2g_reset(self._h, _ptr(obs)))
        else:
            self._check(self._lib.ev2g_reset_ex(self._h, _ptr(obs), int(offset)))

    def _warn_if_general(self):
        if self._spec_checks_left <= 0:
            return
        self._spec_checks_left -= 1
        if self._lib.ev2g_last_launch_specialisation(self._h) == 0:
            why = (self._lib.ev2g_last_launch_general_reason(self._h) or b"").decode()
            quiet = ("EV2G_NO_FULL", "auto_reset", "a cost buffer", "EV2G_FLAG_LOG_CS_HISTORY", "the reward function")
            if why and not why.startswith(quiet):
                self._spec_checks_left = 0
                warnings.warn(f"ev2gym_amd: this launch ran the GENERAL instantiation of {self.kernel_name} (slower than the full one): {why}", stacklevel=3)

    def step(self, actions, obs=None, reward=None, done=None, mask=None):
        self._check(self._lib.ev2g_step(self._h, _ptr(actions), _ptr(obs), _ptr(reward), _ptr(done), _ptr(mask)))
        if self._spec_checks_left > 0:
            self._warn_if_general()

    def step_n(self, k, actions, a_stride, obs=None, o_stride=0, reward=None, r_stride=0, done=None, d_stride=0,
               mask=None, m_stride=0, auto_reset=True, persistent=False):
        rc = self._lib.ev2g_step_n(self._h, int(k), 1 if persistent else 0, _ptr(actions), int(a_stride), _ptr(obs),
# ... 710 lines not shown
```

### include/ev2g.h

```cpp
#ifndef EV2G_H
#define EV2G_H

#include <stddef.h>
#include <stdint.h>

#ifdef __cplusplus
extern "C" {
#endif

#define EV2G_ABI_VERSION 4

#define EV2G_REWARD_PROFITMAX_TRPENALTY_USERINCENTIVES 0
#define EV2G_REWARD_SQUARED_TRACKING_ERROR 1
#define EV2G_REWARD_PROFIT_MAXIMIZATION 2
#define EV2G_REWARD_SQTR_TRPENALTY_USERINCENTIVES 3
#define EV2G_REWARD_SQUARED_TRACKING_ERROR_PENALTY 4
#define EV2G_REWARD_SIMPLE 5
#define EV2G_REWARD_MINIMIZE_TRACKER_SURPLUS 6
#define EV2G_REWARD_V2G_COSTS_SIMPLE 7
#define EV2G_REWARD_V2G_PROFITMAX 8
#define EV2G_REWARD_V2G_PROFITMAX_V2 9
#define EV2G_REWARD_PST_V2G_PROFITMAX_V2 10
#define EV2G_N_REWARDS 11
#define EV2G_STATE_V2G_PROFIT_MAX_LOADS 0
// ... 55 lines not shown

    const double *charge_price;
    const double *discharge_price;
    const double *power_setpoints;

    const double *tr_max_power;
    const double *tr_min_power;
    const double *tr_inflexible_load;
    const double *tr_solar_power;
    const double *tr_load_forecast;
    const double *tr_pv_forecast;
    const double *tr_dr;
    const int32_t *tr_n_dr;
    const int32_t *tr_steps_ahead;

    const int64_t *env_session_start;
    const int32_t *ev_cs;
    const int32_t *ev_t_arr;
    const int32_t *ev_t_dep;
    const int32_t *ev_phases;
    const int32_t *ev_lut;
    const double *ev_cap0;
    const double *ev_B;
    const double *ev_desired;
    const double *ev_minB;
    const double *ev_min_emerg;
    const double *ev_pac_max;
    const double *ev_pac_min;
    const double *ev_pdis_max;
    const double *ev_pdis_min;
    const double *ev_ts;
    const double *ev_tsm;
    const double *ev_eta_ch;
    const double *ev_eta_dis;
    const double *lut;
} ev2g_scenario_batch;

int ev2g_abi_version(void);
int ev2g_create(const ev2g_config *cfg, ev2g_handle **out);
void ev2g_destroy(ev2g_handle *h);
const char *ev2g_last_error(const ev2g_handle *h);

int ev2g_load_scenarios(ev2g_handle *h, const ev2g_scenario_batch *b);

int ev2g_n_envs(const ev2g_handle *h);
int ev2g_n_scenarios(const ev2g_handle *h);
int ev2g_n_ports(const ev2g_handle *h);
int ev2g_obs_dim(const ev2g_handle *h);
int ev2g_n_steps(const ev2g_handle *h);

int ev2g_reset(ev2g_handle *h, double *obs);
int ev2g_reset_ex(ev2g_handle *h, double *obs, int64_t scenario_offset);
int64_t ev2g_scenario_offset(const ev2g_handle *h);

int ev2g_step(ev2g_handle *h, const double *actions, double *obs, double *reward, uint8_t *done,
              uint8_t *action_mask);

#define EV2G_AUTO_RESET_SAME 1
#define EV2G_AUTO_RESET_NEXT 2
#define EV2G_STEPN_PER_STEP_LAUNCH 0
#define EV2G_STEPN_PERSISTENT 1
int ev2g_step_n(ev2g_handle *h, int k_steps, int mode, const double *actions, int64_t action_step_stride,
                double *obs, int64_t obs_step_stride, double *reward, int64_t reward_step_stride,
                uint8_t *done, int64_t done_step_stride, uint8_t *action_mask,
                int64_t mask_step_stride, int auto_reset);

typedef struct ev2g_step_extras {
    double *cost;
    int64_t cost_step_stride;
    float *obs_f32;
    int64_t obs_f32_step_stride;
    const float *actions_f32;
} ev2g_step_extras;
int ev2g_set_step_extras(ev2g_handle *h, const ev2g_step_extras *x);

int ev2g_current_step(const ev2g_handle *h);
const char *ev2g_kernel_name(const ev2g_handle *h);
const char *ev2g_fallback_reason(const ev2g_handle *h);
const char *ev2g_big_kernel_reason(const ev2g_handle *h);
int ev2g_last_launch_specialisation(const ev2g_handle *h);
const char *ev2g_last_launch_general_reason(const ev2g_handle *h);
int ev2g_last_stats_route(const ev2g_handle *h);
const char *ev2g_last_stats_reason(const ev2g_handle *h);
int ev2g_last_launch_fast_forwarded(ev2g_handle *h, int64_t *steps, int64_t *stretches);
int ev2g_check_faults(ev2g_handle *h, int32_t *first_bad_env);

int ev2g_get_stats(ev2g_handle *h, double *stats);
int ev2g_get_stats_reset(ev2g_handle *h, double *stats, double *obs, int64_t scenario_offset);
int ev2g_get_stats_reset_f32(ev2g_handle *h, double *stats, float *obs32, int64_t scenario_offset);
int ev2g_reset_f32(ev2g_handle *h, float *obs32, int64_t scenario_offset);
const char *ev2g_stat_name(int i);

#define EV2G_COMM_ID_BYTES 128
int ev2g_comm_get_unique_id(void *id_out);
int ev2g_comm_init(ev2g_handle *h, const void *id, int rank, int world_size);
void ev2g_comm_destroy(ev2g_handle *h);
int ev2g_comm_world_size(const ev2g_handle *h);
long long ev2g_comm_gathers(const ev2g_handle *h);
int ev2g_gather_stats(ev2g_handle *h, double *stats_all);

typedef struct ev2g_env_view {
    int32_t current_step;
    int32_t n_ports, n_chargers, n_transformers, n_steps;
    double *port_capacity;
    double *port_energy;
    double *port_current;
    double *port_total_energy;
    double *port_required_energy;
    double *port_prev_power;
    int32_t *port_cycles;
    int32_t *port_session;
    double *cs_power;
    double *cs_amps;
    double *cs_profits;
    double *cs_energy_charged;
    double *cs_energy_discharged;
    double *tr_power;
    double *tr_overload;
    double *power_usage;
    double *power_potential;
    int32_t *session_port;
    double *session_afap;
    double *session_final_cap;
} ev2g_env_view;
int ev2g_peek(ev2g_handle *h, int env, ev2g_env_view *view);

typedef struct ev2g_mlp ev2g_mlp;
int ev2g_mlp_create(ev2g_handle *h, int d_in, int h1, int h2, int d_out, const float *W1, const float *b1, const float *W2,
                    const float *b2, const float *W3, const float *b3, float out_lo, ev2g_mlp **out);
#define EV2G_MLP_BF16 0
#define EV2G_MLP_F32 1
#define EV2G_MLP_F32X3 2
int ev2g_mlp_create_ex(ev2g_handle *h, int d_in, int h1, int h2, int d_out, const float *W1, const float *b1, const float *W2,
                    const float *b2, const float *W3, const float *b3, float out_lo, int precision, ev2g_mlp **out);
const char *ev2g_mlp_kernel_name(const ev2g_mlp *m);
void ev2g_mlp_destroy(ev2g_handle *h, ev2g_mlp *m);
int ev2g_mlp_forward(ev2g_handle *h, const ev2g_mlp *m, const float *x, float *y, int n_rows);
int ev2g_rollout(ev2g_handle *h, const ev2g_mlp *m, int k_steps, double *reward, int64_t reward_step_stride, uint8_t *done,
                 int64_t done_step_stride, uint8_t *action_mask, int64_t mask_step_stride, int auto_reset);
long long ev2g_rollout_graph_launches(const ev2g_handle *h);

typedef struct {
    float *obs;
    float *actions;
    double *reward;
    uint8_t *done;
    uint8_t *mask;
} ev2g_transitions;
int ev2g_collect(ev2g_handle *h, const ev2g_mlp *m, int k_steps, const ev2g_transitions *tr);

#define EV2G_HEURISTIC_CHARGE_AS_LATE_AS_POSSIBLE 0
#define EV2G_HEURISTIC_CHARGE_AS_FAST_TO_DESIRED_CAPACITY 1
#define EV2G_HEURISTIC_ROUND_ROBIN 2
#define EV2G_AGENT_CHARGE_AS_LATE_TO_DESIRED_CAPACITY 3
#define EV2G_AGENT_ROUND_ROBIN_GF 4
#define EV2G_AGENT_ROUND_ROBIN_GF_OFF_ALLOWED 5
typedef struct ev2g_heuristic ev2g_heuristic;
int ev2g_heuristic_create(ev2g_handle *h, int kind, ev2g_heuristic **out);
void ev2g_heuristic_destroy(ev2g_handle *h, ev2g_heuristic *a);
int ev2g_heuristic_actions(ev2g_handle *h, ev2g_heuristic *a, double *actions);
int ev2g_heuristic_run(ev2g_handle *h, ev2g_heuristic *a, int k_steps, double *actions, int64_t a_stride, double *obs, int64_t o_stride,
                       double *reward, int64_t r_stride, uint8_t *done, int64_t d_stride, uint8_t *mask, int64_t m_stride);

typedef struct ev2g_link ev2g_link;
int ev2g_link_create(ev2g_handle *h, double p_fail, double p_delay, uint64_t seed_act, uint64_t seed_obs, const double *rand_act,
                     const double *rand_obs, ev2g_link **out);
// ... 252 lines not shown
```

Measured before the change: 1.230 billion env-steps/s.

## Defer tail-group episode stats from persistent step kernel to an end kernel

Adds an opt-in mode where the last-finishing workgroups of the persistent step kernel skip their in-launch episode statistics. They claim a finish rank through a global atomic and record themselves in a list, and a new episode-end kernel recomputes those envs' stats. That kernel gives each env a whole workgroup and stages the SoC log through LDS. The end-of-episode copy and reset is also replaced by this combined kernel, which packs four envs per 256-thread block. The aim is to shorten the step kernel's tail, at the cost of an extra atomic, a sync buffer and more complex host bookkeeping. The deferral fraction defaults to zero.

```diff
diff --git a/ev2gym_amd/csrc/ev2g_device.h b/ev2gym_amd/csrc/ev2g_device.h
--- a/ev2gym_amd/csrc/ev2g_device.h
+++ b/ev2gym_amd/csrc/ev2g_device.h
@@ -959,13 +959,13 @@
 
 #define EV2G_STATS_NK 40
 #define EV2G_STATS_TB 8
+#define EV2G_STAGE_BATCH 16
 #define EV2G_STATS_LK 16
 
-template <int EPWS, int NK, int LK>
-__device__ __forceinline__ void ev2g_env_stats(const StatsView &sv, int e, bool e_valid, int scn, int lane, int cur_step, double *__restrict__ out,
-                                               double *l_keep, int lslot) {
+template <int EPWS>
+__device__ __forceinline__ void ev2g_env_stats_head(const StatsView &sv, int e, bool e_valid, int scn, int lane, int cur_step, double *__restrict__ out) {
     constexpr int W = 64 / EPWS;
-    const int T = sv.T, C = sv.C, R = sv.R, P = sv.P;
+    const int T = sv.T, C = sv.C, R = sv.R;
     double served = 0.0, sat = 0.0, nsat = 0.0;
     for (int c = lane; c < C; c += W) {
         const int n = sv.cs_served[(long long)e * C + c];
@@ -994,6 +994,15 @@
         o[7] = ete;
         o[12] = over;
     }
+}
+
+template <int EPWS, int NK, int LK, bool STAGED = false>
+__device__ __forceinline__ void ev2g_env_stats(const StatsView &sv, int e, bool e_valid, int scn, int lane, int cur_step, double *__restrict__ out,
+                                               double *l_keep, int lslot, int stage_ls = 0) {
+    static_assert(!STAGED || (EPWS == 1 && LK == 0), "the staged variant: one env per workgroup, nothing parked behind the kept entries");
+    constexpr int W = 64 / EPWS;
+    const int T = sv.T, P = sv.P;
+    if (!STAGED) ev2g_env_stats_head<EPWS>(sv, e, e_valid, scn, lane, cur_step, out);
     const double e0 = 7.543e6, e1 = 23.75e6, e2 = 6976, z0 = 7.348e-3, z1 = 3.667, z2 = 7.6e-4, z3 = 4.081e-3;
     const double b_cap_ah = 2.05, b_cap_kwh = 78, d_dist = 15000, b_age = 2 * 365, G_ = 0.186;
     const double theta = 298.15, kk = 0.8263, v_min = 3.3324;
@@ -1015,6 +1024,29 @@
         const bool live = td >= cur_step;
         const double l_cap = sv.line[g].cap, l_abs = sv.line[g].abse;
         const double capk = live ? l_cap : fin_cap;
+        const double *stg = nullptr;
+        if (STAGED) {
+            const int wv = (int)threadIdx.x >> 6;
+            double *row = l_keep + (size_t)lane * stage_ls;
+            __syncthreads();
+            if (log_soc) {
+                const double *__restrict__ slog = sv.soc_log + (long long)e * T * P + q;
+                const int n = spawned ? min(min(td, cur_step - 1) - ta + 1, stage_ls) : 0;
+                const int nw = (n - wv + 3) >> 2;
+                for (int i0 = 0; __any(i0 < nw); i0 += EV2G_STAGE_BATCH) {
+                    double x[EV2G_STAGE_BATCH];
+#pragma unroll
+                    for (int j = 0; j < EV2G_STAGE_BATCH; j++)
+                        x[j] = slog[(long long)min(max(ta + wv + 4 * min(i0 + j, nw - 1), 0), T - 1) * P];
+#pragma unroll
+                    for (int j = 0; j < EV2G_STAGE_BATCH; j++)
+                        if (i0 + j < nw) row[wv + 4 * (i0 + j)] = x[j];
+                }
+            }
+            __syncthreads();
+            if (wv != 0) continue;
+            stg = row - ta;
+        }
         if (spawned) {
             const double v = capk / afap * 100.0;
             sum += v;
@@ -1033,7 +1065,7 @@
                 int n = 0, nf = 0;
                 double xk[NK];
 #pragma unroll
-                for (int u = 0; u < NK; u++) xk[u] = slog[(long long)min(ta + u, tend) * P];
+                for (int u = 0; u < NK; u++) xk[u] = (STAGED ? stg[min(ta + u, tend)] : slog[(long long)min(ta + u, tend) * P]);
 #pragma unroll
                 for (int u = 0; u < NK; u++) {
                     if (ta + u <= tend) {
@@ -1045,7 +1077,7 @@
                 for (int t = ta + NK; t <= tend; t += EV2G_STATS_TB) {
                     double x[EV2G_STATS_TB];
 #pragma unroll
-                    for (int u = 0; u < EV2G_STATS_TB; u++) x[u] = slog[(long long)min(t + u, tend) * P];
+                    for (int u = 0; u < EV2G_STATS_TB; u++) x[u] = (STAGED ? stg[min(t + u, tend)] : slog[(long long)min(t + u, tend) * P]);
                     if (LK > 0 && t - ta - NK < LK) {
 #pragma unroll
                         for (int u = 0; u < EV2G_STATS_TB; u++) l_keep[(t - ta - NK + u) * 64 + lslot] = x[u];
@@ -1073,7 +1105,7 @@
                         for (int u = 0; u < EV2G_STATS_TB; u++) x[u] = l_keep[(t - ta - NK + u) * 64 + lslot];
                     } else {
 #pragma unroll
-                        for (int u = 0; u < EV2G_STATS_TB; u++) x[u] = slog[(long long)min(t + u, tend) * P];
+                        for (int u = 0; u < EV2G_STATS_TB; u++) x[u] = (STAGED ? stg[min(t + u, tend)] : slog[(long long)min(t + u, tend) * P]);
                     }
 #pragma unroll
                     for (int u = 0; u < EV2G_STATS_TB; u++)
@@ -1193,13 +1225,48 @@
     if (RESET && e_valid) ev2g_env_reset<W>(s, st, e, lane, reset_off, r_obs, r_obs32);
 }
 
-template <int EPWS>
-__global__ void __launch_bounds__(64) ev2g_copy_stats_reset_kernel(DevScn s, DevState st, const double *__restrict__ done_stats, double *__restrict__ out,
-                                                                   int reset_off, double *__restrict__ r_obs, float *__restrict__ r_obs32) {
-    constexpr int W = 64 / EPWS;
-    const int sub = threadIdx.x / W, lane = threadIdx.x - sub * W;
-    const int e = blockIdx.x * EPWS + sub;
+#define EV2G_END_BLOCK 256
+#define EV2G_END_STATS_NK 16
+__host__ __device__ inline size_t ev2g_inl_sync_bytes(int n_groups) { return (size_t)(1 + n_groups) * 8 + (size_t)n_groups * 4; }
+__host__ __device__ inline int ev2g_stage_ls(int T) { return T | 1; }
+
+struct EndArgs {
+    const double *ss_afap;
+    double *rows;
+    double *out;
+    const unsigned long long *sync;
+    unsigned long long epoch;
+    int n_heavy;
+    int all_done;
+    int stage_ls;
+    int scn_off, reset_off;
+    double *r_obs; float *r_obs32;
+};
+
+template <bool RESET>
+__global__ void __launch_bounds__(EV2G_END_BLOCK) ev2g_episode_end_kernel(DevScn s, DevState st, EndArgs a) {
+    extern __shared__ double l_stage[];
+    const int wv = (int)threadIdx.x >> 6, lane = (int)threadIdx.x & 63;
+    if ((int)blockIdx.x < a.n_heavy) {
+        const int *list = (const int *)(a.sync + 1 + s.n_groups);
+        const int e = list[(int)blockIdx.x / s.G] * s.G + (int)blockIdx.x % s.G;
+        if (e < 0 || e >= s.E) return;
+        double *dst = RESET ? a.out : a.rows;
+        const StatsView sv = ev2g_stats_view(s, st, a.ss_afap);
+        const int scn = ev2g_scn(e, a.scn_off, s.M);
+        ev2g_env_stats<1, EV2G_END_STATS_NK, 0, true>(sv, e, wv == 0, scn, lane, s.T, dst, l_stage, lane, a.stage_ls);
+        if (wv == 1) ev2g_env_stats_head<1>(sv, e, true, scn, lane, s.T, dst);
+        __syncthreads();
+        if (wv != 0) return;
+        if (!RESET && lane < 17) a.out[(long long)e * 17 + lane] = dst[(long long)e * 17 + lane];
+        if (RESET) ev2g_env_reset<64>(s, st, e, lane, a.reset_off, a.r_obs, a.r_obs32);
+        return;
+    }
+    const int e = ((int)blockIdx.x - a.n_heavy) * (EV2G_END_BLOCK / 64) + wv;
     if (e >= s.E) return;
-    for (int j = lane; j < 17; j += W) out[(long long)e * 17 + j] = done_stats[(long long)e * 17 + j];
-    ev2g_env_reset<W>(s, st, e, lane, reset_off, r_obs, r_obs32);
-}
+    const unsigned long long done = a.all_done ? a.epoch : a.sync[1 + e / s.G];
+    const double v = lane < 17 ? a.rows[(long long)e * 17 + lane] : 0.0;
+    if (done != a.epoch) return;
+    if (lane < 17) a.out[(long long)e * 17 + lane] = v;
+    if (RESET) ev2g_env_reset<64>(s, st, e, lane, a.reset_off, a.r_obs, a.r_obs32);
+}
diff --git a/ev2gym_amd/csrc/ev2g_host.hip b/ev2gym_amd/csrc/ev2g_host.hip
--- a/ev2gym_amd/csrc/ev2g_host.hip
+++ b/ev2gym_amd/csrc/ev2g_host.hip
@@ -184,6 +184,12 @@
     std::vector<double> cs_imax_host;
     int load_gen = 0;
     double *d_stats_inl = nullptr;
+    unsigned long long *d_inl_sync = nullptr;
+    unsigned long long inl_next = 0, inl_epoch = 0;
+    int inl_count = 0;
+    int end_stage_ls = 1;
+    bool inl_rows_complete = false;
+    int last_stats_deferred = 0;
     unsigned long long *d_ff_count = nullptr;
     int last_stats_route = -1;
     const char *stats_reason = "";
@@ -528,6 +534,7 @@
 const char *ev2g_big_kernel_reason(const ev2g_handle *h) { return (h && h->loaded) ? h->big_reason.c_str() : ""; }
 int ev2g_last_launch_specialisation(const ev2g_handle *h) { return (h && h->loaded) ? h->last.specialisation : -1; }
 int ev2g_last_stats_route(const ev2g_handle *h) { return (h && h->loaded) ? h->last_stats_route : -1; }
+int ev2g_last_stats_deferred(const ev2g_handle *h) { return (h && h->loaded) ? h->last_stats_deferred : 0; }
 const char *ev2g_last_stats_reason(const ev2g_handle *h) { return (h && h->loaded && h->last_stats_route == 0) ? h->stats_reason : ""; }
 int ev2g_last_launch_fast_forwarded(ev2g_handle *h, int64_t *steps, int64_t *stretches) {
     if (!h || !h->loaded) return fail(h, EV2G_ERR_STATE, "ev2g_last_launch_fast_forwarded: no scenarios loaded");
@@ -844,9 +851,10 @@
     return upload(h, h->st_allocs, &v2p, 1, &h->d_v2p);
 }
 
-static int load_decide_inl_stats(ev2g_handle *h, const LoadSwitches &sw) {
+static size_t end_stage_bytes(const ev2g_handle *h) { return (size_t)64 * h->end_stage_ls * sizeof(double); }
+static int load_decide_inl_stats(ev2g_handle *h, const LoadPlan &plan, const LoadSwitches &sw) {
     RouteShape &rs = h->shape;
-    h->d_stats_inl = nullptr;
+    h->d_stats_inl = nullptr; h->d_inl_sync = nullptr;
     const char *why = "";
     if (rs.no_inl_stats) why = "EV2G_NO_INLAUNCH_STATS is set";
     else if (!rs.wave() || !(h->cfg.flags & EV2G_FLAG_LOG_SOC)) why = "the step kernel is not ev2g_step_wave with the SoC log";
@@ -865,8 +873,23 @@
         if ((rc = dalloc(h, h->st_allocs, (size_t)h->E * EV2G_N_STATS, &h->d_stats_inl))) return rc;
         double *p = h->d_stats_inl;
         HIPCHK(h, hipMemcpy((char *)h->d_v2p + offsetof(V2P, stats_inl), &p, sizeof p, hipMemcpyHostToDevice));
-    }
+        if ((rc = dalloc(h, h->st_allocs, ev2g_inl_sync_bytes(h->scn.n_groups) / 4, (unsigned **)&h->d_inl_sync))) return rc;
+        unsigned long long *q = h->d_inl_sync;
+        HIPCHK(h, hipMemcpy((char *)h->d_v2p + offsetof(V2P, inl_sync), &q, sizeof q, hipMemcpyHostToDevice));
+    }
+    h->inl_next = 0; h->inl_epoch = 0; h->inl_count = 0; h->inl_rows_complete = false; h->last_stats_deferred = 0;
     rs.ff_count = h->d_ff_count != nullptr; rs.stats_inl = h->d_stats_inl != nullptr;
+    h->end_stage_ls = ev2g_stage_ls((h->cfg.flags & EV2G_FLAG_REFILLABLE) ? h->T : std::min(std::max(plan.longest_stay, 1), h->T));
+    rs.n_groups = h->scn.n_groups;
+    rs.defer_pm = 0; rs.defer_reason = "";
+    if (!rs.stats_inl) rs.defer_reason = "the shape has no in-launch statistics phase";
+    else if (rs.state_kind == EV2G_STATE_PUBLIC_PST) rs.defer_reason = "PublicPST's step kernels do not take a finish rank";
+    else if (end_stage_bytes(h) > 64 * 1024) rs.defer_reason = "the staging block of an env (64 sessions x the longest stay's log entries) does not fit 64 KB of LDS";
+    else rs.defer_pm = sw.inl_stats_defer;
+    if (rs.stats_inl) {
+        const int n = route_inline_count(rs.n_groups, rs.defer_pm);
+        HIPCHK(h, hipMemcpy((char *)h->d_v2p + offsetof(V2P, inl_count), &n, sizeof n, hipMemcpyHostToDevice));
+    }
     return EV2G_OK;
 }
 
@@ -904,7 +927,7 @@
     HIPCHK(h, hipStreamSynchronize(h->stream));
 
     h->E = plan.E; h->M = plan.M; h->scn_off = 0; h->T = plan.T; h->C = plan.C; h->npc = plan.npc; h->P = plan.P; h->R = plan.R; h->D = plan.D; h->S = plan.S;
-    if ((rc = load_decide_inl_stats(h, sw))) return rc;
+    if ((rc = load_decide_inl_stats(h, plan, sw))) return rc;
     h->slot_port = std::move(plan.slot_port);
     h->port_slot = std::move(plan.port_slot);
     h->env_sess_start.assign(b->env_session_start, b->env_session_start + plan.M + 1);
@@ -1012,6 +1035,11 @@
         return fail(h, EV2G_ERR_ARG, r.refusal);
     }
     h->last = r;
+    if (r.inl_stats) {
+        const bool defer = r.inl_count < s.n_groups;
+        if (defer) { h->inl_next += (unsigned long long)s.n_groups; h->inl_epoch = h->inl_next; }
+        h->inl_count = r.inl_count; h->inl_rows_complete = !defer;
+    }
     const V2P *pp = (const V2P *)h->d_v2p;
     const LaunchDims d{dim3(s.n_groups), h->lds_bytes, h->stream};
     switch (r.family) {
@@ -3176,19 +3204,25 @@
     const bool copy = h->last.inl_stats && h->current_step == h->T;
     h->last_stats_route = copy ? 1 : 0;
     h->stats_reason = copy ? "" : h->last.inl_reason;
-    if (copy && !reset) {
-        HIPCHK(h, hipMemcpyAsync(stats, h->d_stats_inl, sizeof(double) * (size_t)h->E * EV2G_N_STATS, hipMemcpyDeviceToDevice, h->stream));
+    h->last_stats_deferred = 0;
+    if (copy) {
+        const int n_def = h->inl_rows_complete ? 0 : h->scn.n_groups - h->inl_count;
+        EndArgs a{};
+        a.ss_afap = h->d_ss_afap; a.rows = h->d_stats_inl; a.out = stats; a.sync = h->d_inl_sync; a.epoch = h->inl_epoch;
+        a.n_heavy = n_def * h->scn.G; a.all_done = h->inl_rows_complete ? 1 : 0; a.stage_ls = h->end_stage_ls;
+        a.scn_off = (int)h->scn_off; a.reset_off = (int)off; a.r_obs = obs; a.r_obs32 = obs32 ? obs32 : (float *)h->extras.obs_f32;
+        const dim3 grid((unsigned)(a.n_heavy + (h->E + EV2G_END_BLOCK / 64 - 1) / (EV2G_END_BLOCK / 64)));
+        const size_t lds = n_def ? end_stage_bytes(h) : 0;
+        if (reset) hipLaunchKernelGGL((ev2g_episode_end_kernel<true>), grid, dim3(EV2G_END_BLOCK), lds, h->stream, h->scn, h->st, a);
+        else hipLaunchKernelGGL((ev2g_episode_end_kernel<false>), grid, dim3(EV2G_END_BLOCK), lds, h->stream, h->scn, h->st, a);
+        HIPCHK(h, hipGetLastError());
+        h->last_stats_deferred = std::min(a.n_heavy, h->E);
+        if (!reset) h->inl_rows_complete = true;
         return EV2G_OK;
     }
 
     const bool pair = stats_pair(h);
     const dim3 grid(pair ? (h->E + 1) / 2 : h->E);
-    if (copy) {
-        hipLaunchKernelGGL((ev2g_copy_stats_reset_kernel<1>), dim3(h->E), dim3(64), 0, h->stream, h->scn, h->st, (const double *)h->d_stats_inl, stats, (int)off, obs,
-                           obs32 ? obs32 : (float *)h->extras.obs_f32);
-        HIPCHK(h, hipGetLastError());
-        return EV2G_OK;
-    }
 #define EV2G_STATS_LAUNCH(EPWS, RESET)                                                                                                    \
     hipLaunchKernelGGL((ev2g_stats_kernel<EPWS, RESET>), grid, dim3(64), (size_t)EV2G_STATS_LK * 64 * sizeof(double), h->stream, h->scn, h->st, (int)h->scn_off, (const double *)h->d_ss_afap, \
                        h->current_step, stats, (int)off, obs, RESET ? (obs32 ? obs32 : (float *)h->extras.obs_f32) : (float *)nullptr)
diff --git a/ev2gym_amd/csrc/ev2g_load_host.h b/ev2gym_amd/csrc/ev2g_load_host.h
--- a/ev2gym_amd/csrc/ev2g_load_host.h
+++ b/ev2gym_amd/csrc/ev2g_load_host.h
@@ -12,10 +12,13 @@
 #include "../../include/ev2g.h"
 #include "ev2g_records.h"
 
+#define EV2G_INL_STATS_DEFER_DEFAULT 0
+
 struct LoadSwitches {
     long long pool_session_cap = 0;
     bool no_full = false, no_wide = false, no_strided = false;
     bool no_inl_stats = false;
+    int inl_stats_defer = EV2G_INL_STATS_DEFER_DEFAULT;
     bool no_fast_forward = false;
     bool kernel_v2 = false;
     bool no_dict = false;
@@ -28,6 +31,7 @@
     sw.no_wide = std::getenv("EV2G_NO_WIDE") != nullptr;
     sw.no_strided = std::getenv("EV2G_NO_STRIDED") != nullptr;
     sw.no_inl_stats = std::getenv("EV2G_NO_INLAUNCH_STATS") != nullptr;
+    if (const char *e = std::getenv("EV2G_INL_STATS_DEFER")) sw.inl_stats_defer = std::min(std::max(std::atoi(e), 0), 1000);
     sw.no_fast_forward = std::getenv("EV2G_NO_FAST_FORWARD") != nullptr;
     const char *kn = std::getenv("EV2G_KERNEL");
     sw.kernel_v2 = kn && std::string(kn) == "v2";
@@ -94,6 +98,7 @@
     std::vector<double> ctab, ptab;
     bool many = false, even = false;
     int tmax = 0, tmin = 0;
+    int longest_stay = 0;
 };
 
 inline int load_plan_check(LoadPlan &p, const ev2g_scenario_batch *b, const ev2g_config &cfg, std::string &msg) {
@@ -329,6 +334,9 @@
     gather(p.ss_emerg, b->ev_min_emerg); gather(p.ss_pacmax, b->ev_pac_max); gather(p.ss_pacmin, b->ev_pac_min);
     gather(p.ss_pdismax, b->ev_pdis_max); gather(p.ss_pdismin, b->ev_pdis_min); gather(p.ss_ts, b->ev_ts); gather(p.ss_tsm, b->ev_tsm);
     gather(p.ss_etach, b->ev_eta_ch); gather(p.ss_etadis, b->ev_eta_dis);
+    p.longest_stay = 0;
+    for (long long d = 0; d < SD; d++)
+        if (dev_to_host[d] >= 0) p.longest_stay = std::max(p.longest_stay, std::min(p.ss_tdep[d], p.T - 1) - p.ss_tarr[d] + 1);
     p.ss_ntarr.assign((size_t)SD, EV2G_INT_MAX); p.ss_ntdep.assign((size_t)SD, EV2G_INT_MAX);
     for (long long d = 0; d + 1 < SD; d++) {
         const long long a = dev_to_host[d], c = dev_to_host[d + 1];
diff --git a/ev2gym_amd/csrc/ev2g_route_host.h b/ev2gym_amd/csrc/ev2g_route_host.h
--- a/ev2gym_amd/csrc/ev2g_route_host.h
+++ b/ev2gym_amd/csrc/ev2g_route_host.h
@@ -21,6 +21,8 @@
     bool ff_count = false;
     bool stats_inl = false;
     const char *inl_shape_reason = "";
+    int n_groups = 0, defer_pm = 0;
+    const char *defer_reason = "";
     bool wave() const { return family == ROUTE_WAVE; }
     bool big() const { return family == ROUTE_BIG; }
 };
@@ -42,6 +44,7 @@
     int specialisation = -1;
     bool ff = false;
     bool inl_stats = false;
+    int inl_count = 0;
     const char *general_reason = "";
     const char *inl_reason = "";
     const char *refusal = nullptr;
@@ -53,6 +56,11 @@
 constexpr int route_wave_index(int sk, int rk, bool io32, int fullk) { return ((sk * 4 + rk) * 2 + (io32 ? 1 : 0)) * 4 + fullk; }
 constexpr bool route_wave_exists(int sk, int rk, bool io32, int fullk) {
     return sk >= 0 && sk < 3 && rk >= 0 && rk < 4 && fullk >= 0 && fullk < 4 && (fullk == 0 || (rk != 3 && (fullk != 3 || !io32)));
+}
+
+inline int route_inline_count(int n_groups, int defer_pm) {
+    const long long pm = std::min(std::max(defer_pm, 0), 1000);
+    return n_groups - (int)((long long)n_groups * pm / 1000);
 }
 
 inline StepRoute route_step(const RouteShape &s, const RouteCall &c) {
@@ -100,6 +108,7 @@
         else if (!s.stats_inl) r.inl_reason = s.inl_shape_reason;
         else r.inl_reason = "";
         r.inl_stats = r.inl_reason[0] == 0;
+        r.inl_count = r.inl_stats ? route_inline_count(s.n_groups, s.defer_pm) : 0;
         return r;
     }
     const bool v2 = s.family == ROUTE_V2 || s.family == ROUTE_BIG;
diff --git a/ev2gym_amd/csrc/ev2g_step_v2.h b/ev2gym_amd/csrc/ev2g_step_v2.h
--- a/ev2gym_amd/csrc/ev2g_step_v2.h
+++ b/ev2gym_amd/csrc/ev2g_step_v2.h
@@ -135,6 +135,8 @@
     EV2G_GP(const double) ss_B; EV2G_GP(const double) ss_afap;
     EV2G_GP(double) stats_inl;
     EV2G_GP(unsigned long long) ff_count;
+    EV2G_GP(unsigned long long) inl_sync;
+    int inl_count, inl_pad;
     EV2G_GP(double) x_cost; long long x_c_stride;
     EV2G_GP(float) x_obs32; long long x_o32_stride;
     EV2G_GP(const float) x_act32;
@@ -159,7 +161,7 @@
     CPS(price_ch) CPS(price_dis) CPS(setpoint) CPS(tr_infl) CPS(tr_solar) CPS(tr_base) CPS(tr_maxp) CPS(tr_minp)
     CPS(win_tab) CPS(lut) CPS(rec) CPS(tail) CPS(ss_lut) CPS(sess_dyn) CPS(cls_rec)
     CPS(scn_sess) CPS(scn_sess_end) CPS(ss_slot) CPS(ss_tarr) CPS(ss_tdep) CPS(ss_B)
-    EV2G_SETP(p.ss_afap, (const double *)nullptr); EV2G_SETP(p.stats_inl, (double *)nullptr); EV2G_SETP(p.ff_count, (unsigned long long *)nullptr);
+    EV2G_SETP(p.ss_afap, (const double *)nullptr); EV2G_SETP(p.stats_inl, (double *)nullptr); EV2G_SETP(p.ff_count, (unsigned long long *)nullptr); EV2G_SETP(p.inl_sync, (unsigned long long *)nullptr); p.inl_count = 0x7fffffff; p.inl_pad = 0;
     CPT(line) CPT(cs_sat_sum) CPT(cs_served)
     CPT(cs_profits) CPT(cs_e_ch) CPT(cs_e_dis) CPT(cs_power_hist) CPT(cs_cur_hist) CPT(cs_power_now) CPT(cs_cur_now)
     CPT(env_acc) CPT(env_fault) CPT(hist) CPT(tr_power_now)
diff --git a/ev2gym_amd/csrc/ev2g_step_wave.h b/ev2gym_amd/csrc/ev2g_step_wave.h
--- a/ev2gym_amd/csrc/ev2g_step_wave.h
+++ b/ev2gym_amd/csrc/ev2g_step_wave.h
@@ -944,9 +944,22 @@
     PT_FLUSH
     double *stats_out = (INL && t == T && k_steps > 1) ? (double *)S->stats_inl : nullptr;
     if (stats_out != nullptr) {
+        const int n_grp = (S->E + BLOCK / 64 - 1) / (BLOCK / 64), inl_count = S->inl_count;
+        const bool defer = SK != 1 && inl_count < n_grp;
+        if (defer && tid == 0) {
+            typedef unsigned long long __attribute__((address_space(1))) *SyncPtr;
+            const SyncPtr sync = (SyncPtr)S->inl_sync;
+            const int b = (int)blockIdx.x, grp_s = (n_grp & 7) == 0 ? (b & 7) * (n_grp >> 3) + (b >> 3) : b;
+            const unsigned long long r = __hip_atomic_fetch_add(sync, 1ull, __ATOMIC_RELAXED, __HIP_MEMORY_SCOPE_AGENT);
+            const int rank = (int)(r % (unsigned long long)n_grp), slot = rank - inl_count;
+            items[0] = slot;
+            if (slot < 0) sync[1 + grp_s] = r - (unsigned long long)rank + (unsigned long long)n_grp;
+            else if (slot < n_grp) ((int __attribute__((address_space(1))) *)(sync + 1 + n_grp))[slot] = grp_s;
+        }
         __syncthreads();
+        const int slot = defer ? __builtin_amdgcn_readfirstlane(items[0]) : -1;
         const int es = e0 + wv;
-        if (es < S->E) {
+        if (slot < 0 && es < S->E) {
             const int scn_s = (int)(__builtin_amdgcn_readfirstlane(hb_step) / (64u * (unsigned)T));
             StatsView v{T, S->C, S->R, P, S->dt, (const double *)S->setpoint, (const int *)S->scn_sess, (const int *)S->scn_sess_end,
                         (const int *)S->ss_slot, (const int *)S->ss_tarr, (const int *)S->ss_tdep, (const double *)S->ss_B, (const double *)S->ss_afap,
diff --git a/ev2gym_amd/engine.py b/ev2gym_amd/engine.py
--- a/ev2gym_amd/engine.py
+++ b/ev2gym_amd/engine.py
@@ -52,6 +52,7 @@
         "ev2g_last_launch_general_reason": (C.c_char_p, [vp]),
         "ev2g_last_stats_route": (C.c_int, [vp]),
         "ev2g_last_stats_reason": (C.c_char_p, [vp]),
+        "ev2g_last_stats_deferred": (C.c_int, [vp]),
         "ev2g_last_launch_fast_forwarded": (C.c_int, [vp, C.POINTER(C.c_int64), C.POINTER(C.c_int64)]),
         "ev2g_fallback_reason": (C.c_char_p, [vp]),
         "ev2g_big_kernel_reason": (C.c_char_p, [vp]),
@@ -207,7 +208,7 @@
 EXPORTED_SYMBOLS = [
     "ev2g_abi_version", "ev2g_create", "ev2g_destroy", "ev2g_last_error", "ev2g_load_scenarios", "ev2g_n_envs",
     "ev2g_n_scenarios", "ev2g_n_ports", "ev2g_obs_dim", "ev2g_n_steps", "ev2g_current_step", "ev2g_reset", "ev2g_reset_ex",
-    "ev2g_scenario_offset", "ev2g_set_step_extras", "ev2g_kernel_name", "ev2g_last_launch_specialisation", "ev2g_last_launch_general_reason", "ev2g_last_stats_route", "ev2g_last_stats_reason", "ev2g_last_launch_fast_forwarded", "ev2g_fallback_reason", "ev2g_big_kernel_reason", "ev2g_step", "ev2g_step_n",
+    "ev2g_scenario_offset", "ev2g_set_step_extras", "ev2g_kernel_name", "ev2g_last_launch_specialisation", "ev2g_last_launch_general_reason", "ev2g_last_stats_route", "ev2g_last_stats_reason", "ev2g_last_stats_deferred", "ev2g_last_launch_fast_forwarded", "ev2g_fallback_reason", "ev2g_big_kernel_reason", "ev2g_step", "ev2g_step_n",
     "ev2g_check_faults", "ev2g_get_stats", "ev2g_get_stats_reset", "ev2g_get_stats_reset_f32", "ev2g_reset_f32", "ev2g_collect", "ev2g_stat_name", "ev2g_peek", "ev2g_malloc", "ev2g_free",
     "ev2g_memcpy_h2d", "ev2g_memcpy_d2h", "ev2g_host_malloc", "ev2g_host_free", "ev2g_synchronize", "ev2g_fill_uniform", "ev2g_host_uniform",
     "ev2g_last_step_n_kernel_ms", "ev2g_step_n_kernel_ms_back", "ev2g_mlp_create", "ev2g_mlp_create_ex", "ev2g_mlp_destroy", "ev2g_mlp_forward", "ev2g_mlp_kernel_name", "ev2g_rollout",
@@ -318,6 +319,10 @@
     @property
     def last_stats_route(self) -> int:
         return int(self._lib.ev2g_last_stats_route(self._h))
+
+    @property
+    def last_stats_deferred(self) -> int:
+        return int(self._lib.ev2g_last_stats_deferred(self._h))
 
     @property
     def last_stats_reason(self) -> str:
diff --git a/include/ev2g.h b/include/ev2g.h
--- a/include/ev2g.h
+++ b/include/ev2g.h
@@ -161,6 +161,7 @@
 const char *ev2g_last_launch_general_reason(const ev2g_handle *h);
 int ev2g_last_stats_route(const ev2g_handle *h);
 const char *ev2g_last_stats_reason(const ev2g_handle *h);
+int ev2g_last_stats_deferred(const ev2g_handle *h);
 int ev2g_last_launch_fast_forwarded(ev2g_handle *h, int64_t *steps, int64_t *stretches);
 int ev2g_check_faults(ev2g_handle *h, int32_t *first_bad_env);
 
```

After: 1.226 billion env-steps/s. No clear change (-0.3%).
